# rs-anderson/explicit-alignment-for-vqa-tasks

Hardware: AMD Instinct MI355X
Metric: mapper_train_samples_per_sec (higher is better)
Workload: dtype bf16; 1 GPU; cfg2: CLIP ViT-B/32 -> GPT-2-large (774M), MLP mapper, prefix 10, CC-shaped synthetic batches; per-GPU batch 64, S=42; fwd+bwd+AdamW; random-init weights; global_batch=64, seq_len=42, parallelism=dp1

## Files before the change

### explicit-alignment-for-vqa-tasks_amd/_lib.py

```python
from __future__ import annotations

import ctypes as C
import os

_HERE = os.path.dirname(os.path.abspath(__file__))
LIB_PATH = os.path.join(_HERE, "csrc", "libeavqa_hip.so")

F32, BF16 = 0, 1
ACT = {"none": 0, "tanh": 1, "relu": 2, "gelu_new": 3, "quick_gelu": 4}

i32, i64, f32, ptr = C.c_int, C.c_int64, C.c_float, C.c_void_p

SIGNATURES = {
    "eavqa_abi_version": [],
    "eavqa_strerror": [i32],
    "eavqa_check_device": [],
    "eavqa_gemm": [i32, i32, i32, i32, i32, i32, ptr, i64, ptr, i64, ptr, i64, i32, f32, ptr, i32, ptr, ptr, i64, ptr, i64, ptr],
    "eavqa_layernorm_fwd": [i32, i32, i32, i32, ptr, i64, ptr, ptr, f32, ptr, i64, ptr, ptr, ptr],
    "eavqa_layernorm_bwd": [i32, i32, i32, i32, ptr, i64, ptr, i64, ptr, ptr, ptr, ptr, ptr, i64, ptr, ptr, ptr, i64, ptr],
    "eavqa_layernorm_fwd_fp8": [i32, i32, i32, ptr, i64, ptr, ptr, f32, ptr, i64, ptr, ptr, ptr, ptr],
    "eavqa_layernorm_bwd_fp8": [i32, i32, i32, ptr, i64, ptr, i64, ptr, ptr, ptr, ptr, ptr, i64, ptr, i64, ptr, ptr],
    "eavqa_attention_fwd": [i32, i32, i32, i32, i32, i32, ptr, i64, ptr, i64, ptr, i64, ptr, i64, i64, i64, ptr, i64, ptr, i32, f32, ptr, ptr],
    "eavqa_attention_decode": [i32, i32, i32, i32, i32, ptr, i64, ptr, i64, ptr, i64, i64, ptr, ptr, i64, ptr, i64, ptr, i64, f32, ptr],
    "eavqa_attention_decode_splitk": [i32, i32, i32, i32, i32, ptr, i32, ptr, ptr, i64, ptr, i64, i64, ptr, i64, ptr, i64, f32, ptr],
    "eavqa_attention_bwd": [i32, i32, i32, i32, i32, i32, ptr, i64, ptr, i64, ptr, i64, ptr, i64, ptr, i64,
                            ptr, i64, ptr, i64, ptr, i64, ptr, ptr, i32, f32, ptr, ptr, ptr],
    "eavqa_build_prefix_rows": [i32, i32, i32, ptr, ptr, i32, i32, i32, ptr, ptr, ptr, ptr],
    "eavqa_build_fewshot_rows": [i32, i32, i32, i32, i64, ptr, ptr, i32, ptr, ptr, ptr, ptr, ptr],
    "eavqa_build_row_plan": [i32, i32, i32, ptr, ptr, ptr, ptr, ptr, ptr, ptr, ptr, ptr, ptr],
    "eavqa_copy_rows": [i32, i32, i32, i32, ptr, i64, i64, ptr, i64, i64, i64, ptr],
    "eavqa_transpose": [i32, i32, i32, ptr, i64, ptr, i64, ptr],
    "eavqa_select_rows": [i32, ptr, i32, ptr, ptr, ptr, ptr],
    "eavqa_move_rows": [i32, i32, i32, i32, ptr, i64, ptr, ptr, i64, ptr],
    "eavqa_l2_normalize_rows": [i32, i32, ptr, i64, ptr],
    "eavqa_topk_rows": [i32, i32, ptr, i64, i32, ptr, ptr, ptr],
    "eavqa_gemm_splitk_plan": [i32, i32, i32],
    "eavqa_gemm_splitk": [i32, i32, i32, i32, ptr, i64, ptr, i64, ptr, i32, ptr],
    "eavqa_splitk_finish": [i32, i32, i32, ptr, i32, ptr, i32, ptr, i64, i32, i32, ptr, i64, ptr, i64, ptr, i64, ptr],
    "eavqa_layernorm_splitk": [i32, i32, i32, ptr, i64, ptr, i32, ptr, ptr, i64, ptr, ptr, f32, ptr, i64, ptr],
    "eavqa_gemm_fp8_splitk_plan": [i32, i32, i32],
    "eavqa_gemm_fp8_splitk": [i32, i32, i32, ptr, i64, ptr, ptr, i64, f32, ptr, i32, ptr],
    "eavqa_layernorm_splitk_fp8": [i32, i32, ptr, i64, ptr, i32, ptr, ptr, i64, ptr, ptr, f32, ptr, i64, ptr, ptr],
    "eavqa_rmsnorm_splitk": [i32, i32, i32, ptr, i64, ptr, i32, ptr, i64, ptr, f32, ptr, i64, ptr],
    "eavqa_splitk_finish_gated": [i32, i32, i32, ptr, i32, i32, ptr, i64, ptr],
    "eavqa_attention_decode_splitk_rel": [i32, i32, i32, i32, i32, ptr, i32, i32, ptr, i64, ptr, i64, i64, ptr, i64, ptr, i64, f32, ptr, i64, i32, ptr],
    "eavqa_colsum": [i32, i32, i32, ptr, i64, ptr, i32, ptr],
    "eavqa_embed_assemble": [i32, i32, i32, ptr, ptr, ptr, i64, ptr, i64, ptr, i64, ptr, i64, ptr],
    "eavqa_embed_assemble_bwd": [i32, i32, i32, ptr, ptr, i64, ptr, i64, ptr],
    "eavqa_build_labels": [i32, i32, i32, i32, ptr, i64, i64, ptr, ptr],
    "eavqa_ce_fwd": [i32, i32, i32, ptr, i64, ptr, ptr, ptr, ptr, ptr, ptr],
    "eavqa_guard_count": [ptr, i32, ptr, ptr],
    "eavqa_ce_bwd": [i32, i32, i32, i32, ptr, i64, ptr, ptr, ptr, ptr, ptr, i64, ptr],
    "eavqa_greedy_pick": [i32, i32, ptr, i64, i64, i64, ptr, ptr, i64, ptr, ptr, ptr, ptr],
    "eavqa_adamw": [i64, ptr, ptr, ptr, ptr, i32, f32, f32, f32, f32, f32, f32, i32, ptr, ptr],
    "eavqa_patchify": [i32, i32, i32, i32, ptr, ptr, i64, ptr],
    "eavqa_vit_assemble": [i32, i32, i32, i32, ptr, i64, ptr, ptr, ptr, i64, ptr],
    "eavqa_cast_rows": [i32, i32, i64, ptr, i64, ptr, i64, ptr],
    "eavqa_quantize_rows_fp8": [i32, i32, i32, ptr, i64, ptr, i64, ptr, ptr],
    "eavqa_rmsnorm_fwd": [i32, i32, i32, i32, ptr, i64, ptr, f32, ptr, i64, ptr, ptr],
    "eavqa_rmsnorm_bwd": [i32, i32, i32, i32, ptr, i64, ptr, i64, ptr, ptr, ptr, ptr, i64, ptr, i64, ptr],
    "eavqa_gated_act_fwd": [i32, i32, i32, i32, ptr, i64, ptr, i64, ptr],
    "eavqa_gated_act_bwd": [i32, i32, i32, i32, ptr, i64, ptr, i64, ptr, i64, ptr],
    "eavqa_attention_fwd_rel": [i32, i32, i32, i32, i32, i32, ptr, i64, ptr, i64, ptr, i64, ptr, i64, i64, i64, ptr, i64, i32, f32, ptr, i64, i32, ptr, ptr],
    "eavqa_attention_bwd_rel": [i32, i32, i32, i32, i32, i32, ptr, i64, ptr, i64, ptr, i64, ptr, i64, ptr, i64, ptr, i64, ptr, i64, ptr, i64,
                                ptr, i32, f32, ptr, i64, i32, ptr, ptr, ptr],
    "eavqa_gemm_fp8": [i32, i32, i32, ptr, i64, ptr, ptr, i64, f32, ptr, i64, i32, f32, ptr, i32, ptr, ptr, i64, ptr, i64, ptr, i32],
}
class LMLayer(C.Structure):
    _fields_ = [(n, C.c_void_p) for n in ("ln1_g", "ln1_b", "w_qkv", "b_qkv", "w_o", "b_o", "ln2_g", "ln2_b", "w_fc1", "b_fc1",
                                          "w_fc2", "b_fc2", "k_cache", "v_cache")]


class LMLayerScales(C.Structure):
    _fields_ = [(n, C.c_float) for n in ("s_qkv", "s_o", "s_fc1", "s_fc2")]


class T5DecLayer(C.Structure):
    _fields_ = [(n, C.c_void_p) for n in ("ln_sa", "w_qkv", "w_o", "ln_ca", "w_q_ca", "w_o_ca", "ln_ff", "w_i", "w_o_ff", "k_cache", "v_cache",
                                          "cross_kv")]


class DecodeGemm(C.Structure):
    _fields_ = [("M", i32), ("N", i32), ("K", i32), ("A", ptr), ("lda", i64), ("a_kind", i32), ("gamma", ptr), ("beta", ptr), ("eps", f32),
                ("stats_in", ptr), ("n_stats_in", i32), ("stats_in_cols", i32), ("B", ptr), ("ldb", i64), ("gated_rows", i32),
                ("bias", ptr), ("act", i32), ("residual", ptr), ("ld_residual", i64), ("out_f32", i32), ("n_seg", i32),
                ("out", ptr * 3), ("ld_out", i64 * 3), ("stats_out", ptr)]


class GemmLn(C.Structure):
    _fields_ = [("copy_out", ptr), ("ld_copy", i64), ("stats_out", ptr), ("stats_ld", i32), ("ln_stats", ptr), ("ln_parts", i32),
                ("ln_ld", i32), ("ln_cols", i32), ("ln_c", ptr), ("ln_eps", f32), ("mean_out", ptr), ("rstd_out", ptr)]


SIGNATURES["eavqa_gemm_ln"] = SIGNATURES["eavqa_gemm"][:-1] + [C.POINTER(GemmLn), ptr]
SIGNATURES["eavqa_gemm_decode_cols"] = [i32, i32, i32, i32, i32]
SIGNATURES["eavqa_gemm_decode"] = [C.POINTER(DecodeGemm), ptr]
SIGNATURES["eavqa_t5_decoder_step_workspace_bytes"] = [i32, i32, i32, i32, i32, i32]
SIGNATURES["eavqa_t5_decoder_step"] = [i32, i32, C.POINTER(T5DecLayer), ptr, i32, i32, i32, i32, i32, i32, f32, i32, i32, i32, i32, ptr, ptr, ptr, i64,
                                       ptr, i64, i32, ptr, i64, ptr]
SIGNATURES["eavqa_lm_block_workspace_bytes"] = [i32, i32, i32, i32]
SIGNATURES["eavqa_lm_block_fp8_workspace_bytes"] = [i32, i32, i32]
SIGNATURES["eavqa_lm_block_forward_fp8"] = [i32, C.POINTER(LMLayer), C.POINTER(LMLayerScales), i32, i32, i32, i32, f32, i32, i32, i32, i32, ptr, ptr, i64, ptr, i64, ptr]
SIGNATURES["eavqa_lm_block_forward"] = [i32, i32, C.POINTER(LMLayer), i32, i32, i32, i32, f32, i32, i32, i32, i32, ptr, ptr, i64, ptr, i64, ptr]

SIGNATURES["eavqa_gemm_ex"] = SIGNATURES["eavqa_gemm"] + [i32]
SIGNATURES["eavqa_gemm_ln_ex"] = SIGNATURES["eavqa_gemm_ln"] + [i32]
SIGNATURES["eavqa_attention_fwd_ex"] = SIGNATURES["eavqa_attention_fwd"] + [i32]
SIGNATURES["eavqa_attention_bwd_ex"] = SIGNATURES["eavqa_attention_bwd"] + [i32]
SIGNATURES["eavqa_gemm_splitk_ex"] = SIGNATURES["eavqa_gemm_splitk"] + [i32]
SIGNATURES["eavqa_lm_block_forward_ex"] = SIGNATURES["eavqa_lm_block_forward"] + [i32]
SIGNATURES["eavqa_gemm_decode_ex"] = SIGNATURES["eavqa_gemm_decode"] + [i32]
SIGNATURES["eavqa_t5_decoder_step_ex"] = SIGNATURES["eavqa_t5_decoder_step"] + [i32]

_RESTYPES = {"eavqa_strerror": C.c_char_p, "eavqa_lm_block_workspace_bytes": C.c_int64, "eavqa_lm_block_fp8_workspace_bytes": C.c_int64, "eavqa_t5_decoder_step_workspace_bytes": C.c_int64}

_lib = None


class EavqaError(RuntimeError):
    pass


def load() -> C.CDLL:
    global _lib
    if _lib is not None:
        return _lib
    if not os.path.exists(LIB_PATH):
        raise EavqaError(
            f"{LIB_PATH} is missing: the HIP extension is the only compute path. "
            "Build it with `python -m eavqa_amd.build` (needs hipcc, no GPU required to compile)."
        )
    import torch
    lib = C.CDLL(LIB_PATH)
    for name, argtypes in SIGNATURES.items():
        fn = getattr(lib, name)
        fn.argtypes = argtypes
        fn.restype = _RESTYPES.get(name, C.c_int)
    got = lib.eavqa_abi_version()
    if got != 1:
        raise EavqaError(f"libeavqa_hip.so ABI version {got}, host code expects 1")
    _lib = lib
    return lib


def call(name: str, *args) -> None:
    lib = load()
    rc = getattr(lib, name)(*args)
    if rc != 0:
        raise EavqaError(f"{name} failed: {lib.eavqa_strerror(rc).decode()} (code {rc})")
```

### explicit-alignment-for-vqa-tasks_amd/build.py

```python
from __future__ import annotations

import hashlib
import json
import os
import shutil
import subprocess
import sys
from concurrent.futures import ThreadPoolExecutor

PKG_DIR = os.path.dirname(os.path.abspath(__file__))
CSRC = os.path.join(PKG_DIR, "csrc")
ROOT = os.path.dirname(PKG_DIR)
INCLUDE = os.path.join(ROOT, "include")
OBJ = os.path.join(CSRC, "_obj")
LIB = os.path.join(CSRC, "libeavqa_hip.so")
EXPORTS = os.path.join(CSRC, "exports.map")

HIP_SOURCES = ["gemm.hip", "norm.hip", "attention.hip", "seq.hip", "loss.hip", "optim.hip", "decode.hip", "decode_direct.hip", "retrieval.hip"]
CPP_SOURCES = ["api.cpp", "lm_block.cpp", "t5_block.cpp"]
ARCH = "gfx950"


def _hipcc() -> str:
    exe = shutil.which("hipcc") or "/opt/rocm/bin/hipcc"
    if not os.path.exists(exe):
        raise RuntimeError("hipcc not found: libeavqa_hip.so cannot be built")
    return exe


def _newer(dst: str, deps) -> bool:
    if not os.path.exists(dst):
        return False
    t = os.path.getmtime(dst)
    return all(os.path.getmtime(d) <= t for d in deps)


FLAGS = ["-O3", "-std=c++17", "-fPIC", "-Xarch_host", "-fvisibility=hidden"]


def _digest(rel_paths, extra: str) -> str:
    h = hashlib.sha256(extra.encode())
    for p in rel_paths:
        h.update(p.encode())
        with open(os.path.join(ROOT, p), "rb") as f:
            h.update(f.read())
    return h.hexdigest()


def _read_deps(dfile: str):
    with open(dfile) as f:
        text = f.read().replace("\\\n", " ")
    deps = [os.path.abspath(t) for t in text.split(":", 1)[1].split()]
    return sorted({os.path.relpath(d, ROOT) for d in deps if d.startswith(ROOT + os.sep)})


def _compile(src: str, verbose: bool) -> str:
    stem = os.path.splitext(src)[0]
    obj, dfile, kfile = (os.path.join(OBJ, stem + ext) for ext in (".o", ".d", ".key.json"))
    path = os.path.join(CSRC, src)
    flags = FLAGS + [f"--offload-arch={ARCH}"] + ([] if src.endswith(".hip") else ["-x", "hip"])
    cmd = [_hipcc()] + flags + [f"-I{INCLUDE}", f"-I{CSRC}", "-MD", "-MF", dfile, "-c", path, "-o", obj]
    if os.path.exists(obj) and os.path.exists(kfile):
        try:
            with open(kfile) as f:
                key = json.load(f)
            if key["digest"] == _digest(key["deps"], " ".join(flags)):
                return obj
        except (OSError, KeyError, ValueError):
            pass
    if verbose:
        print(" ".join(cmd), flush=True)
    r = subprocess.run(cmd, capture_output=True, text=True)
    if r.returncode != 0:
        raise RuntimeError(f"hipcc failed on {src}:\n{r.stdout}\n{r.stderr}")
    deps = _read_deps(dfile)
    with open(kfile, "w") as f:
        json.dump({"deps": deps, "digest": _digest(deps, " ".join(flags))}, f)
    return obj


def build(verbose: bool = False, force: bool = False) -> str:
    os.makedirs(OBJ, exist_ok=True)
    if force:
        for f in os.listdir(OBJ):
            os.remove(os.path.join(OBJ, f))
    srcs = HIP_SOURCES + CPP_SOURCES
    with ThreadPoolExecutor(max_workers=min(4, len(srcs))) as ex:
        objs = list(ex.map(lambda s: _compile(s, verbose), srcs))
    if not _newer(LIB, objs + [EXPORTS]):
        cmd = [_hipcc(), f"--offload-arch={ARCH}", "-shared", "-fPIC", f"-Wl,--version-script={EXPORTS}", "-o", LIB] + objs
        if verbose:
            print(" ".join(cmd), flush=True)
        r = subprocess.run(cmd, capture_output=True, text=True)
        if r.returncode != 0:
            raise RuntimeError(f"link failed:\n{r.stdout}\n{r.stderr}")
    return LIB


if __name__ == "__main__":
    print(build(verbose=True, force="--force" in sys.argv))
```

### explicit-alignment-for-vqa-tasks_amd/csrc/gemm.hip

```cpp
#include "common.h"

namespace {

struct Knobs {
    int stagger;
    int ablate;
    bool disable_fast;
    int k64_mode;
    int big_mode;
    int deep;
    int shape_mode;
    int group_n;
    bool no_row_split;
    explicit Knobs(int k = 0) : stagger(k & 15), ablate((k >> 4) & 7), disable_fast(((k >> 7) & 1) != 0), k64_mode((k >> 8) & 63),
                                big_mode((k >> 14) & 3), deep((k >> 16) & 3), shape_mode((k >> 18) & 7), group_n((k >> 21) & 15),
                                no_row_split(((k >> 25) & 1) != 0) {}
};

struct GemmParamsBase {
    const void* A; const void* B; void* C;
    const float* bias; const void* aux_in; void* aux_out; const void* residual;
    const float* row_scale;
    int M, N, K;
    int64_t lda, ldb, ldc, ld_aux, ldr;
    int act, out_f32, res_lowp;
    int out_f16;
    int ablate;
    float alpha;
    int tiles_m, tiles_n;
    int group_n;
    int vec_c, vec_aux, vec_res, vec_bias;
};
struct GemmParams : GemmParamsBase {
    void* copy_out = nullptr; int64_t ld_copy = 0; int vec_copy = 0;
    float* stats_out = nullptr; int stats_ld = 0;
    const float* ln_stats = nullptr; int ln_parts = 0, ln_ld = 0;
    const float* ln_c = nullptr; float ln_inv_n = 0.f, ln_eps = 0.f;
    float* mean_out = nullptr; float* rstd_out = nullptr;
};
constexpr int LN_ROWSTAT_BYTES = 2048;
inline int ln_lds(const GemmParams& p) { return p.ln_stats ? LN_ROWSTAT_BYTES : 0; }
__device__ __forceinline__ GemmParams widen(const GemmParams& k) { return k; }
__device__ __forceinline__ GemmParams widen(const GemmParamsBase& k) { GemmParams p; static_cast<GemmParamsBase&>(p) = k; return p; }
template <bool LNX> struct KernArg { using type = GemmParamsBase; };
template <> struct KernArg<true> { using type = GemmParams; };

constexpr int BM = 128, BN = 128;
constexpr int CS_PITCH = 132;
constexpr int CS_BYTES = BM * CS_PITCH * 4;

__device__ __forceinline__ void tile_coords(const GemmParams& p, int& tm, int& tn) {
    const int nwg = p.tiles_m * p.tiles_n;
    const int bid = blockIdx.x;
    const int q = nwg >> 3, r = nwg & 7, xcd = bid & 7;
    const int wgid = (xcd < r ? xcd * (q + 1) : r * (q + 1) + (xcd - r) * q) + (bid >> 3);
    tm = wgid % p.tiles_m;
    tn = wgid / p.tiles_m;
}

__device__ __forceinline__ void ln_rowstat_fill(const GemmParams& p, float2* rowstat, int m0, int n0, int rows, int tid, int nthreads) {
    if (!p.ln_stats) return;
    for (int r = tid; r < rows; r += nthreads) {
        const int m = min(m0 + r, p.M - 1);
        const float2* q = reinterpret_cast<const float2*>(p.ln_stats) + (int64_t)m * p.ln_ld;
        float s = 0.f, ss = 0.f;
        if (((p.ln_ld | p.ln_parts) & 1) == 0 && (reinterpret_cast<uintptr_t>(p.ln_stats) & 15) == 0) {
            const float4* q4 = reinterpret_cast<const float4*>(q);
            const int n4 = p.ln_parts >> 1;
            for (int i = 0; i < n4; i += 4) {
                float4 t[4];
#pragma unroll
                for (int k = 0; k < 4; ++k) t[k] = q4[min(i + k, n4 - 1)];
#pragma unroll
                for (int k = 0; k < 4; ++k) {
                    const float w = (i + k < n4) ? 1.f : 0.f;
                    s += w * (t[k].x + t[k].z);
                    ss += w * (t[k].y + t[k].w);
                }
            }
        } else {
            for (int i = 0; i < p.ln_parts; ++i) { const float2 t = q[i]; s += t.x; ss += t.y; }
        }
        const float mean = s * p.ln_inv_n;
        const float rstd = 1.0f / sqrtf(fmaxf(ss * p.ln_inv_n - mean * mean, 0.f) + p.ln_eps);
        rowstat[r] = make_float2(rstd, -rstd * mean);
        if (n0 == 0 && m0 + r < p.M && p.mean_out) { p.mean_out[m] = mean; p.rstd_out[m] = rstd; }
    }
}

template <int TPR_, int RPP_, int NPASS_, int PITCH_, int ROWS_ = RPP_ * NPASS_, int LN_UNROLL_ = 4> struct EpiGeo {
    static constexpr int TPR = TPR_, RPP = RPP_, NPASS = NPASS_, PITCH = PITCH_, ROWS = ROWS_;
    static constexpr int LN_UNROLL = LN_UNROLL_;
};
using EpiGeo128 = EpiGeo<32, 8, 16, CS_PITCH>;

template <typename T, int ACT, int MODE, bool FULL, bool LNX>
__device__ __forceinline__ void epilogue_quad(const GemmParams& p, int m, int n, float (&v)[4], const float (&bias4)[4], const float2 rs,
                                              const float (&c4)[4]) {
    const T* aux_in = reinterpret_cast<const T*>(p.aux_in);
    T* aux_out = reinterpret_cast<T*>(p.aux_out);
    const bool full = FULL || (n + 3 < p.N);
    const float al = p.row_scale ? p.alpha * p.row_scale[m] : p.alpha;
    if (LNX && p.ln_stats) {
#pragma unroll
        for (int j = 0; j < 4; ++j) v[j] = (al * rs.x) * v[j] + (bias4[j] + rs.y * c4[j]);
    } else {
#pragma unroll
        for (int j = 0; j < 4; ++j) v[j] = al * v[j] + bias4[j];
    }
    if (aux_out) {
        T* q = aux_out + (int64_t)m * p.ld_aux + n;
        if (FULL || (full && p.vec_aux)) elem<T>::st4(q, make_float4(v[0], v[1], v[2], v[3]));
        else
            for (int j = 0; j < 4; ++j)
                if (n + j < p.N) elem<T>::st(q + j, v[j]);
    }
    if (MODE == 2) {
        const T* q = aux_in + (int64_t)m * p.ld_aux + n;
        float u[4] = {0.f, 0.f, 0.f, 0.f};
        if (FULL || (full && p.vec_aux)) { float4 t = elem<T>::ld4(q); u[0] = t.x; u[1] = t.y; u[2] = t.z; u[3] = t.w; }
        else
            for (int j = 0; j < 4; ++j)
                if (n + j < p.N) u[j] = elem<T>::ld(q + j);
#pragma unroll
        for (int j = 0; j < 4; ++j) v[j] *= act_bwd(ACT, u[j]);
    } else if (MODE == 1) {
#pragma unroll
        for (int j = 0; j < 4; ++j) v[j] = act_fwd(ACT, v[j]);
    }
    if (p.residual) {
        if (p.res_lowp == 2) {
            const f16_t* q = reinterpret_cast<const f16_t*>(p.residual) + (int64_t)m * p.ldr + n;
            if (FULL || (full && p.vec_res)) { float4 t = elem<f16_t>::ld4(q); v[0] += t.x; v[1] += t.y; v[2] += t.z; v[3] += t.w; }
            else
                for (int j = 0; j < 4; ++j)
                    if (n + j < p.N) v[j] += elem<f16_t>::ld(q + j);
        } else if (p.res_lowp) {
            const T* q = reinterpret_cast<const T*>(p.residual) + (int64_t)m * p.ldr + n;
            if (FULL || (full && p.vec_res)) { float4 t = elem<T>::ld4(q); v[0] += t.x; v[1] += t.y; v[2] += t.z; v[3] += t.w; }
            else
                for (int j = 0; j < 4; ++j)
                    if (n + j < p.N) v[j] += elem<T>::ld(q + j);
        } else {
            const float* q = reinterpret_cast<const float*>(p.residual) + (int64_t)m * p.ldr + n;
            if (FULL || (full && p.vec_res)) { float4 t = *reinterpret_cast<const float4*>(q); v[0] += t.x; v[1] += t.y; v[2] += t.z; v[3] += t.w; }
            else
                for (int j = 0; j < 4; ++j)
                    if (n + j < p.N) v[j] += q[j];
        }
    }
    if (p.out_f32) {
        float* q = reinterpret_cast<float*>(p.C) + (int64_t)m * p.ldc + n;
        if (FULL || (full && p.vec_c)) *reinterpret_cast<float4*>(q) = make_float4(v[0], v[1], v[2], v[3]);
        else
            for (int j = 0; j < 4; ++j)
                if (n + j < p.N) q[j] = v[j];
    } else if (p.out_f16) {
        f16_t* q = reinterpret_cast<f16_t*>(p.C) + (int64_t)m * p.ldc + n;
        if (FULL || (full && p.vec_c)) elem<f16_t>::st4(q, make_float4(v[0], v[1], v[2], v[3]));
        else
            for (int j = 0; j < 4; ++j)
                if (n + j < p.N) elem<f16_t>::st(q + j, v[j]);
    } else {
        T* q = reinterpret_cast<T*>(p.C) + (int64_t)m * p.ldc + n;
        if (FULL || (full && p.vec_c)) elem<T>::st4(q, make_float4(v[0], v[1], v[2], v[3]));
        else
            for (int j = 0; j < 4; ++j)
                if (n + j < p.N) elem<T>::st(q + j, v[j]);
    }
    if (LNX && p.copy_out) {
        T* q = reinterpret_cast<T*>(p.copy_out) + (int64_t)m * p.ld_copy + n;
        if (full && p.vec_copy) elem<T>::st4(q, make_float4(v[0], v[1], v[2], v[3]));
        else
            for (int j = 0; j < 4; ++j)
                if (n + j < p.N) elem<T>::st(q + j, v[j]);
    }
}

template <bool FULL>
__device__ __forceinline__ void load_bias4(const GemmParams& p, int n, float (&bias4)[4]) {
    bias4[0] = bias4[1] = bias4[2] = bias4[3] = 0.f;
    if (p.bias) {
        if (FULL) { const float4 b = *reinterpret_cast<const float4*>(p.bias + n); bias4[0] = b.x; bias4[1] = b.y; bias4[2] = b.z; bias4[3] = b.w; }
        else {
#pragma unroll
            for (int j = 0; j < 4; ++j)
                if (n + j < p.N) bias4[j] = p.bias[n + j];
        }
    }
}

struct LnArgs { const float2* rowstat; int row_base; };

template <typename T, int ACT, int MODE, bool FULL, typename G, bool LNX>
__device__ __forceinline__ void epilogue_body(const GemmParams& p, float* Cs, int m0, int n0, const LnArgs ln) {
    const int tid = threadIdx.x;
    if (G::ROWS != G::RPP * G::NPASS && tid >= G::TPR * G::RPP) return;
    const int c4 = (tid % G::TPR) * 4;
    const int n = n0 + c4;
    float bias4[4], lc4[4] = {0.f, 0.f, 0.f, 0.f};
    load_bias4<FULL>(p, n, bias4);
    if (LNX && p.ln_stats) {
#pragma unroll
        for (int j = 0; j < 4; ++j)
            if (FULL || n + j < p.N) lc4[j] = p.ln_c[n + j];
    }
    auto one_pass = [&](int pass) {
        const int row = (tid / G::TPR) + pass * G::RPP;
        const int m = m0 + row;
        if (G::ROWS != G::RPP * G::NPASS && row >= G::ROWS) return;
        if (!FULL && (m >= p.M || n >= p.N)) return;
        const float4 a = *reinterpret_cast<const float4*>(&Cs[row * G::PITCH + c4]);
        float v[4] = {a.x, a.y, a.z, a.w};
        const float2 rs = (LNX && p.ln_stats) ? ln.rowstat[ln.row_base + row] : make_float2(1.f, 0.f);
        epilogue_quad<T, ACT, MODE, FULL, LNX>(p, m, n, v, bias4, rs, lc4);
        if (LNX && p.stats_out) {
            if (!FULL) {
#pragma unroll
                for (int j = 0; j < 4; ++j)
                    if (n + j >= p.N) v[j] = 0.f;
            }
            *reinterpret_cast<float4*>(&Cs[row * G::PITCH + c4]) = make_float4(v[0], v[1], v[2], v[3]);
        }
    };
    if constexpr (LNX && G::LN_UNROLL == 1) {
#pragma unroll 1
        for (int pass = 0; pass < G::NPASS; ++pass) one_pass(pass);
    } else {
#pragma unroll 4
        for (int pass = 0; pass < G::NPASS; ++pass) one_pass(pass);
    }
}

template <typename G>
__device__ __forceinline__ void epilogue_row_sums(const GemmParams& p, const float* Cs, int m0, int n0) {
    constexpr int COLS = G::TPR * 4;
    static_assert(COLS >= 64 && COLS % 4 == 0, "a tile covers at least one 64-column slot");
    __syncthreads();
    const int cols = min(COLS, p.N - n0);
    const int slot0 = n0 / 64, slot1 = (n0 + COLS < p.N) ? (n0 + COLS) / 64 : p.stats_ld;
    for (int r = threadIdx.x; r < G::ROWS; r += blockDim.x) {
        const int m = m0 + r;
        if (m >= p.M) continue;
        float s = 0.f, ss = 0.f;
        for (int c = 0; c < cols; c += 4) {
            const float4 t = *reinterpret_cast<const float4*>(&Cs[r * G::PITCH + c]);
            s += (t.x + t.y) + (t.z + t.w);
            ss += (t.x * t.x + t.y * t.y) + (t.z * t.z + t.w * t.w);
        }
        float2* q = reinterpret_cast<float2*>(p.stats_out) + (int64_t)m * p.stats_ld;
        q[slot0] = make_float2(s, ss);
        for (int i = slot0 + 1; i < slot1; ++i) q[i] = make_float2(0.f, 0.f);
    }
}

template <typename T, int ACT, int MODE, typename G, bool LNX>
__device__ __forceinline__ void epilogue_mode(const GemmParams& p, float* Cs, int m0, int n0, const LnArgs ln) {
    constexpr int ROWS = G::ROWS, COLS = G::TPR * 4;
    const bool full_tile = (m0 + ROWS <= p.M) && (n0 + COLS <= p.N) && p.vec_c && (!(p.aux_in || p.aux_out) || p.vec_aux) &&
                           (!p.residual || p.vec_res) && (!p.bias || p.vec_bias);
    if (full_tile) epilogue_body<T, ACT, MODE, true, G, LNX>(p, Cs, m0, n0, ln);
    else epilogue_body<T, ACT, MODE, false, G, LNX>(p, Cs, m0, n0, ln);
    if (LNX && p.stats_out) epilogue_row_sums<G>(p, Cs, m0, n0);
}

template <typename T, typename G = EpiGeo128, bool LNX = true>
__device__ __forceinline__ void epilogue(const GemmParams& p, float* Cs, int m0, int n0, const LnArgs ln = LnArgs{nullptr, 0}) {
    const int mode = p.aux_in ? 2 : (p.act != EAVQA_ACT_NONE ? 1 : 0);
    if (mode == 0) { epilogue_mode<T, EAVQA_ACT_NONE, 0, G, LNX>(p, Cs, m0, n0, ln); return; }
    switch (p.act) {
        case EAVQA_ACT_TANH:
            if (mode == 1) epilogue_mode<T, EAVQA_ACT_TANH, 1, G, LNX>(p, Cs, m0, n0, ln); else epilogue_mode<T, EAVQA_ACT_TANH, 2, G, LNX>(p, Cs, m0, n0, ln);
            break;
        case EAVQA_ACT_RELU:
            if (mode == 1) epilogue_mode<T, EAVQA_ACT_RELU, 1, G, LNX>(p, Cs, m0, n0, ln); else epilogue_mode<T, EAVQA_ACT_RELU, 2, G, LNX>(p, Cs, m0, n0, ln);
            break;
        case EAVQA_ACT_GELU_NEW:
            if (mode == 1) epilogue_mode<T, EAVQA_ACT_GELU_NEW, 1, G, LNX>(p, Cs, m0, n0, ln); else epilogue_mode<T, EAVQA_ACT_GELU_NEW, 2, G, LNX>(p, Cs, m0, n0, ln);
            break;
        case EAVQA_ACT_QUICK_GELU:
            if (mode == 1) epilogue_mode<T, EAVQA_ACT_QUICK_GELU, 1, G, LNX>(p, Cs, m0, n0, ln); else epilogue_mode<T, EAVQA_ACT_QUICK_GELU, 2, G, LNX>(p, Cs, m0, n0, ln);
            break;
        default:
            epilogue_mode<T, EAVQA_ACT_NONE, 0, G, LNX>(p, Cs, m0, n0, ln);
    }
}

template <typename T, typename G = EpiGeo128>
__device__ __forceinline__ void epilogue_any(const GemmParams& p, float* Cs, int m0, int n0, const LnArgs ln = LnArgs{nullptr, 0}) {
    if (p.ln_stats || p.stats_out || p.copy_out) epilogue<T, G, true>(p, Cs, m0, n0, ln);
    else epilogue<T, G, false>(p, Cs, m0, n0, ln);
}


constexpr int BK16 = 64;
constexpr int OPER16_BYTES = 128 * BK16 * 2;

__device__ __forceinline__ int swz16(int row, int kc) { return row * 128 + ((kc ^ (row & 7)) << 4); }

template <bool KC>
__device__ __forceinline__ void g2r_16(uint4 (&r)[4], const bf16_t* X, int64_t ld, int row0, int rows_max,
                                       int k0, int K) {
    const int tid = threadIdx.x;
#pragma unroll
    for (int i = 0; i < 4; ++i) {
        const int c = tid + 256 * i;
        uint4 v = make_uint4(0u, 0u, 0u, 0u);
        if (KC) {
            const int row = c >> 3, kc = c & 7;
            const int gr = row0 + row, gk = k0 + kc * 8;
            if (gr < rows_max && gk < K) v = *reinterpret_cast<const uint4*>(X + (int64_t)gr * ld + gk);
        } else {
            const int k = c >> 4, rc = c & 15;
            const int gk = k0 + k, gr = row0 + rc * 8;
            if (gk < K && gr < rows_max) v = *reinterpret_cast<const uint4*>(X + (int64_t)gk * ld + gr);
        }
        r[i] = v;
    }
}
template <bool KC>
__device__ __forceinline__ void r2s_16(const uint4 (&r)[4], char* S) {
    const int tid = threadIdx.x;
#pragma unroll
    for (int i = 0; i < 4; ++i) {
        const int c = tid + 256 * i;
        if (KC) {
// ... 612 lines not shown
inline int big_grid(int tiles_m, int tiles_n, int& gx, int& gy) {
    int best_gx = 8, best_cost = 1 << 30, best_rounds = 1 << 30;
    const int cand[4] = {8, 4, 2, 1};
    for (int c = 0; c < 4; ++c) {
        const int x = cand[c], y = 8 / x;
        const int pm = (tiles_m + x - 1) / x, pn = (tiles_n + y - 1) / y;
        const int rounds = (pm * pn + 31) / 32, cost = pm + pn;
        if (rounds < best_rounds || (rounds == best_rounds && cost < best_cost)) { best_rounds = rounds; best_cost = cost; best_gx = x; }
    }
    gx = best_gx; gy = 8 / gx;
    return ((tiles_m + gx - 1) / gx) * ((tiles_n + gy - 1) / gy);
}

int launch_big(const GemmParams& p, hipStream_t stream) {
    static std::atomic<bool> configured{false};
    if (!configured.load(std::memory_order_acquire)) {
        if (hipFuncSetAttribute(reinterpret_cast<const void*>(gemm_bf16_big_kernel<false>), hipFuncAttributeMaxDynamicSharedMemorySize,
                                GLDS_BYTES) != hipSuccess ||
            hipFuncSetAttribute(reinterpret_cast<const void*>(gemm_bf16_big_kernel<true>), hipFuncAttributeMaxDynamicSharedMemorySize,
                                GLDS_BYTES + LN_ROWSTAT_BYTES) != hipSuccess)
            return EAVQA_E_LAUNCH;
        configured.store(true, std::memory_order_release);
    }
    const int tiles_m = (p.M + GBM - 1) / GBM, tiles_n = (p.N + GBN - 1) / GBN;
    int gx, gy;
    const int per_xcd = big_grid(tiles_m, tiles_n, gx, gy);
    if (p.ln_stats || p.stats_out || p.copy_out)
        hipLaunchKernelGGL(gemm_bf16_big_kernel<true>, dim3(per_xcd * 8), dim3(1024), GLDS_BYTES + ln_lds(p), stream, p, gx, gy, tiles_m, tiles_n);
    else
        hipLaunchKernelGGL(gemm_bf16_big_kernel<false>, dim3(per_xcd * 8), dim3(1024), GLDS_BYTES, stream, p, gx, gy, tiles_m, tiles_n);
    EAVQA_LAUNCH_CHECK();
    return EAVQA_OK;
}

inline int big_split_rows(int M, int N) {
    const int rem = M % GBM;
    if (rem == 0 || rem > 192 || M <= GBM) return 0;
    int gx, gy;
    const int tiles_n = (N + GBN - 1) / GBN;
    const int with = (big_grid((M + GBM - 1) / GBM, tiles_n, gx, gy) + 31) / 32, without = (big_grid(M / GBM, tiles_n, gx, gy) + 31) / 32;
    return without < with ? rem : 0;
}

bool use_big(const GemmParams& p, const Knobs& kn) {
    if (p.K % GBK) return false;
    if (kn.big_mode == 1) return false;
    if (kn.big_mode == 2) return true;
    const int tiles = ((p.M + GBM - 1) / GBM) * ((p.N + GBN - 1) / GBN);
    return tiles >= 144;
}


#include "gemm_k64.hip"

inline float k64_cost(const GemmParams& p, const K64Choice& c, float* multi_round_loop = nullptr) {
    const int tiles_m = (p.M + c.bm - 1) / c.bm, tiles_n = (p.N + c.bn - 1) / c.bn;
    const GridPlan g = plan_grid(tiles_m, tiles_n, c.bm, c.bn);
    const float rounds = float((g.per_xcd + 31) / 32);
    const float loop = rounds * c.rate * (c.bm + c.bn) * (p.K / 64);
    if (multi_round_loop) *multi_round_loop = rounds > 1.f ? loop : 0.f;
    return loop + rounds * 0.1f * c.bm * c.bn + 4500.f;
}

#include "gemm_fp8.hip"

template <int MF>
__global__ __launch_bounds__(512) void gemm_bf16_skinny_kernel(GemmParams p) {
    __shared__ float red[8][64][17];
    const int tid = threadIdx.x, lane = tid & 63, wave = tid >> 6;
    const int x = lane & 15, g = lane >> 4;
    const int n0 = blockIdx.x * 16;
    const bf16_t* A = reinterpret_cast<const bf16_t*>(p.A);
    const bf16_t* B = reinterpret_cast<const bf16_t*>(p.B);
    const int nsteps = p.K >> 5;
    const int per_wave = (nsteps + 7) >> 3;
    const int s_begin = wave * per_wave, s_end = min(nsteps, s_begin + per_wave);
    const bf16_t* bp = B + (int64_t)min(n0 + x, p.N - 1) * p.ldb + 8 * g;
    const bf16_t* ap[MF];
#pragma unroll
    for (int f = 0; f < MF; ++f) ap[f] = A + (int64_t)min(16 * f + x, p.M - 1) * p.lda + 8 * g;
    f32x4 acc[MF];
#pragma unroll
    for (int f = 0; f < MF; ++f) acc[f] = (f32x4){0.f, 0.f, 0.f, 0.f};

    int s = s_begin;
    for (; s + 8 <= s_end; s += 8) {
        bf16x8 b[8], a[8][MF];
#pragma unroll
        for (int u = 0; u < 8; ++u) {
            b[u] = *reinterpret_cast<const bf16x8*>(bp + (s + u) * 32);
#pragma unroll
            for (int f = 0; f < MF; ++f) a[u][f] = *reinterpret_cast<const bf16x8*>(ap[f] + (s + u) * 32);
        }
#pragma unroll
        for (int u = 0; u < 8; ++u)
#pragma unroll
            for (int f = 0; f < MF; ++f) acc[f] = __builtin_amdgcn_mfma_f32_16x16x32_bf16(a[u][f], b[u], acc[f], 0, 0, 0);
    }
    for (; s < s_end; ++s) {
        const bf16x8 b = *reinterpret_cast<const bf16x8*>(bp + s * 32);
#pragma unroll
        for (int f = 0; f < MF; ++f) {
            const bf16x8 a = *reinterpret_cast<const bf16x8*>(ap[f] + s * 32);
            acc[f] = __builtin_amdgcn_mfma_f32_16x16x32_bf16(a, b, acc[f], 0, 0, 0);
        }
    }
#pragma unroll
    for (int f = 0; f < MF; ++f)
#pragma unroll
        for (int r = 0; r < 4; ++r) red[wave][16 * f + 4 * g + r][x] = acc[f][r];
    __syncthreads();
    for (int e = tid; e < MF * 16 * 16; e += 512) {
        const int m = e >> 4, c = e & 15, n = n0 + c;
        if (m >= p.M || n >= p.N) continue;
        float v = 0.f;
#pragma unroll
        for (int w = 0; w < 8; ++w) v += red[w][m][c];
        v = p.alpha * v + (p.bias ? p.bias[n] : 0.f);
        const int64_t ia = (int64_t)m * p.ld_aux + n;
        if (p.aux_out) elem<bf16_t>::st(reinterpret_cast<bf16_t*>(p.aux_out) + ia, v);
        if (p.aux_in) v *= act_bwd(p.act, elem<bf16_t>::ld(reinterpret_cast<const bf16_t*>(p.aux_in) + ia));
        else v = act_fwd(p.act, v);
        if (p.residual) v += p.res_lowp == 2 ? elem<f16_t>::ld(reinterpret_cast<const f16_t*>(p.residual) + (int64_t)m * p.ldr + n)
                             : p.res_lowp ? elem<bf16_t>::ld(reinterpret_cast<const bf16_t*>(p.residual) + (int64_t)m * p.ldr + n)
                                          : reinterpret_cast<const float*>(p.residual)[(int64_t)m * p.ldr + n];
        if (p.out_f32) reinterpret_cast<float*>(p.C)[(int64_t)m * p.ldc + n] = v;
        else if (p.out_f16) elem<f16_t>::st(reinterpret_cast<f16_t*>(p.C) + (int64_t)m * p.ldc + n, v);
        else elem<bf16_t>::st(reinterpret_cast<bf16_t*>(p.C) + (int64_t)m * p.ldc + n, v);
    }
}

int launch_skinny(const GemmParams& p, hipStream_t stream) {
    const int blocks = (p.N + 15) / 16;
    const int mf = (p.M + 15) / 16;
    if (mf == 1) hipLaunchKernelGGL(gemm_bf16_skinny_kernel<1>, dim3(blocks), dim3(512), 0, stream, p);
    else if (mf == 2) hipLaunchKernelGGL(gemm_bf16_skinny_kernel<2>, dim3(blocks), dim3(512), 0, stream, p);
    else if (mf == 3) hipLaunchKernelGGL(gemm_bf16_skinny_kernel<3>, dim3(blocks), dim3(512), 0, stream, p);
    else hipLaunchKernelGGL(gemm_bf16_skinny_kernel<4>, dim3(blocks), dim3(512), 0, stream, p);
    EAVQA_LAUNCH_CHECK();
    return EAVQA_OK;
}

constexpr int BK32 = 16;
constexpr int PITCH32 = 17;
constexpr int OPER32_FLOATS = 128 * PITCH32;

template <bool KC>
__device__ __forceinline__ void g2r_32(float4 (&r)[2], const float* X, int64_t ld, int row0, int rows_max,
                                       int k0, int K) {
    const int tid = threadIdx.x;
#pragma unroll
    for (int i = 0; i < 2; ++i) {
        const int c = tid + 256 * i;
        float4 v = make_float4(0.f, 0.f, 0.f, 0.f);
        if (KC) {
            const int row = c >> 2, kc = c & 3;
            const int gr = row0 + row, gk = k0 + kc * 4;
            if (gr < rows_max && gk < K) v = *reinterpret_cast<const float4*>(X + (int64_t)gr * ld + gk);
        } else {
            const int k = c >> 5, rc = c & 31;
            const int gk = k0 + k, gr = row0 + rc * 4;
            if (gk < K && gr < rows_max) v = *reinterpret_cast<const float4*>(X + (int64_t)gk * ld + gr);
        }
        r[i] = v;
    }
}
template <bool KC>
__device__ __forceinline__ void r2s_32(const float4 (&r)[2], float* S) {
    const int tid = threadIdx.x;
#pragma unroll
    for (int i = 0; i < 2; ++i) {
        const int c = tid + 256 * i;
        const float w[4] = {r[i].x, r[i].y, r[i].z, r[i].w};
        if (KC) {
            const int row = c >> 2, kc = c & 3;
#pragma unroll
            for (int j = 0; j < 4; ++j) S[row * PITCH32 + kc * 4 + j] = w[j];
        } else {
            const int k = c >> 5, rc = c & 31;
#pragma unroll
            for (int j = 0; j < 4; ++j) S[(rc * 4 + j) * PITCH32 + k] = w[j];
        }
    }
}

template <bool A_KC, bool B_KC>
__global__ __launch_bounds__(256) void gemm_f32_kernel(GemmParams p) {
    extern __shared__ __attribute__((aligned(16))) char smem[];
    float* sm = reinterpret_cast<float*>(smem);
    float* const As0 = sm;
    float* const Bs0 = sm + 2 * OPER32_FLOATS;

    int tm, tn;
    tile_coords(p, tm, tn);
    const int m0 = tm * BM, n0 = tn * BN;
    const int tid = threadIdx.x, lane = tid & 63, wave = tid >> 6;
    const int wm = wave >> 1, wn = wave & 1;
    const float* A = reinterpret_cast<const float*>(p.A);
    const float* B = reinterpret_cast<const float*>(p.B);

    f32x16 acc[2][2];
#pragma unroll
    for (int i = 0; i < 2; ++i)
#pragma unroll
        for (int j = 0; j < 2; ++j)
#pragma unroll
            for (int r = 0; r < 16; ++r) acc[i][j][r] = 0.f;

    const int nk = (p.K + BK32 - 1) / BK32;
    float4 ra[2], rb[2];
    g2r_32<A_KC>(ra, A, p.lda, m0, p.M, 0, p.K);
    g2r_32<B_KC>(rb, B, p.ldb, n0, p.N, 0, p.K);
    r2s_32<A_KC>(ra, As0);
    r2s_32<B_KC>(rb, Bs0);
    __syncthreads();

    const int frow = lane & 31, fk = lane >> 5;
    for (int kt = 0; kt < nk; ++kt) {
        const int cur = kt & 1;
        if (kt + 1 < nk) {
            g2r_32<A_KC>(ra, A, p.lda, m0, p.M, (kt + 1) * BK32, p.K);
            g2r_32<B_KC>(rb, B, p.ldb, n0, p.N, (kt + 1) * BK32, p.K);
        }
        const float* Ac = As0 + cur * OPER32_FLOATS;
        const float* Bc = Bs0 + cur * OPER32_FLOATS;
#pragma unroll
        for (int s = 0; s < BK32 / 2; ++s) {
            float af[2], bfr[2];
#pragma unroll
            for (int i = 0; i < 2; ++i) af[i] = Ac[(wm * 64 + i * 32 + frow) * PITCH32 + s * 2 + fk];
#pragma unroll
            for (int j = 0; j < 2; ++j) bfr[j] = Bc[(wn * 64 + j * 32 + frow) * PITCH32 + s * 2 + fk];
#pragma unroll
            for (int i = 0; i < 2; ++i)
#pragma unroll
                for (int j = 0; j < 2; ++j)
                    acc[i][j] = __builtin_amdgcn_mfma_f32_32x32x2f32(af[i], bfr[j], acc[i][j], 0, 0, 0);
        }
        if (kt + 1 < nk) {
            r2s_32<A_KC>(ra, As0 + (cur ^ 1) * OPER32_FLOATS);
            r2s_32<B_KC>(rb, Bs0 + (cur ^ 1) * OPER32_FLOATS);
        }
        __syncthreads();
    }

    float* Cs = reinterpret_cast<float*>(smem);
#pragma unroll
    for (int i = 0; i < 2; ++i)
#pragma unroll
        for (int j = 0; j < 2; ++j)
#pragma unroll
            for (int r = 0; r < 16; ++r) {
                const int row = wm * 64 + i * 32 + (r & 3) + 8 * (r >> 2) + 4 * (lane >> 5);
                const int col = wn * 64 + j * 32 + (lane & 31);
                Cs[row * CS_PITCH + col] = acc[i][j][r];
            }
    float2* rowstat = reinterpret_cast<float2*>(smem + CS_BYTES);
    ln_rowstat_fill(p, rowstat, m0, n0, BM, tid, 256);
    __syncthreads();
    if constexpr (A_KC && B_KC) epilogue_any<float>(p, Cs, m0, n0, LnArgs{rowstat, 0});
    else epilogue<float, EpiGeo128, false>(p, Cs, m0, n0);
}

typedef void (*gemm_kernel_t)(GemmParams);

int launch(gemm_kernel_t kernel, const GemmParams& p, hipStream_t stream) {
    static std::atomic<gemm_kernel_t> configured[8];
    bool done = false;
    for (int i = 0; i < 8; ++i) done |= (configured[i].load(std::memory_order_acquire) == kernel);
    if (!done) {
        if (hipFuncSetAttribute(reinterpret_cast<const void*>(kernel), hipFuncAttributeMaxDynamicSharedMemorySize,
                                CS_BYTES + LN_ROWSTAT_BYTES) != hipSuccess)
            return EAVQA_E_LAUNCH;
        for (int i = 0; i < 8; ++i) {
            gemm_kernel_t expected = nullptr;
            if (configured[i].compare_exchange_strong(expected, kernel, std::memory_order_acq_rel) || expected == kernel) break;
        }
    }
    const int nwg = p.tiles_m * p.tiles_n;
    hipLaunchKernelGGL(kernel, dim3(nwg), dim3(256), CS_BYTES + ln_lds(p), stream, p);
    EAVQA_LAUNCH_CHECK();
    return EAVQA_OK;
}


}

namespace {
eavqa_gemm_ln_t ln_rows_from(const eavqa_gemm_ln_t& x, int64_t r0, size_t esz) {
    eavqa_gemm_ln_t y = x;
    if (x.copy_out) y.copy_out = static_cast<char*>(x.copy_out) + (size_t)r0 * (size_t)x.ld_copy * esz;
    if (x.stats_out) y.stats_out = x.stats_out + (size_t)r0 * (size_t)x.stats_ld * 2;
    if (x.ln_stats) y.ln_stats = x.ln_stats + (size_t)r0 * (size_t)x.ln_ld * 2;
    if (x.mean_out) y.mean_out = x.mean_out + r0;
    if (x.rstd_out) y.rstd_out = x.rstd_out + r0;
    return y;
}

int gemm_impl(int dtype, int a_kc, int b_kc, int M, int N, int K,
              const void* A, int64_t lda, const void* B, int64_t ldb,
              void* C, int64_t ldc, int out_flags, float alpha,
              const float* bias, int act,
              const void* aux_in, void* aux_out, int64_t ld_aux,
              const void* residual, int64_t ldr, const eavqa_gemm_ln_t* ln, void* stream, int knobs) {
    const Knobs kn(knobs);
    const bool ln_consumer = ln && ln->ln_stats;
    if (ln) {
        if (ln->copy_out && ln->ld_copy < N) return EAVQA_E_ARG;
        if (ln->stats_out && ln->stats_ld < (N + 63) / 64) return EAVQA_E_ARG;
        if (ln_consumer && (!ln->ln_c || ln->ln_parts <= 0 || ln->ln_ld < ln->ln_parts || ln->ln_cols <= 0 || !(ln->ln_eps >= 0.f))) return EAVQA_E_ARG;
        if ((ln->mean_out != nullptr) != (ln->rstd_out != nullptr) || (ln->mean_out && !ln_consumer)) return EAVQA_E_ARG;
        if (!(a_kc && b_kc)) return EAVQA_E_SHAPE;
    }
    if (out_flags & ~(EAVQA_GEMM_OUT_F32 | EAVQA_GEMM_RESIDUAL_LOWP | EAVQA_GEMM_STREAM_F16)) return EAVQA_E_ARG;
    if ((out_flags & (EAVQA_GEMM_RESIDUAL_LOWP | EAVQA_GEMM_STREAM_F16)) && dtype != EAVQA_BF16) return EAVQA_E_DTYPE;
    const int out_f32 = out_flags & EAVQA_GEMM_OUT_F32;
    const int stream_f16 = (out_flags & EAVQA_GEMM_STREAM_F16) != 0;
    const int res_lowp = (out_flags & EAVQA_GEMM_RESIDUAL_LOWP) ? (stream_f16 ? 2 : 1) : 0;
    if (!A || !B || !C) return EAVQA_E_ARG;
    if (M <= 0 || N <= 0 || K <= 0) return EAVQA_E_ARG;
    if (dtype != EAVQA_F32 && dtype != EAVQA_BF16) return EAVQA_E_DTYPE;
    if (act < EAVQA_ACT_NONE || act > EAVQA_ACT_QUICK_GELU) return EAVQA_E_DTYPE;
    const int vec = dtype == EAVQA_BF16 ? 8 : 4;
    const int a_contig = a_kc ? K : M, b_contig = b_kc ? K : N;
    if (a_contig % vec || b_contig % vec) return EAVQA_E_SHAPE;
    if (lda % vec || ldb % vec) return EAVQA_E_ALIGN;
    if (!eavqa_aligned16(A) || !eavqa_aligned16(B)) return EAVQA_E_ALIGN;
    if (lda < a_contig || ldb < b_contig || ldc < N) return EAVQA_E_ARG;
    if ((aux_in || aux_out) && ld_aux < N) return EAVQA_E_ARG;
    if (residual && ldr < N) return EAVQA_E_ARG;

    GemmParams p;
    p.A = A; p.B = B; p.C = C; p.bias = bias; p.aux_in = aux_in; p.aux_out = aux_out; p.residual = residual; p.row_scale = nullptr; p.ablate = kn.ablate;
    p.M = M; p.N = N; p.K = K; p.lda = lda; p.ldb = ldb; p.ldc = ldc; p.ld_aux = ld_aux; p.ldr = ldr;
    p.act = act; p.out_f32 = out_f32; p.res_lowp = res_lowp; p.out_f16 = stream_f16 && !out_f32; p.alpha = alpha;
    p.group_n = kn.group_n == 0 ? BIG_GROUP_N : kn.group_n - 1;
    p.tiles_m = (M + BM - 1) / BM;
    p.tiles_n = (N + BN - 1) / BN;
    const int esz = dtype == EAVQA_BF16 ? 2 : 4;
    auto vec_ok = [](const void* ptr, int64_t ld, int bytes_per_elem) {
        return ((reinterpret_cast<uintptr_t>(ptr) % (4 * bytes_per_elem)) == 0) && (ld % 4 == 0);
    };
    p.vec_c = vec_ok(C, ldc, out_f32 ? 4 : esz);
    p.vec_aux = vec_ok(aux_in ? aux_in : aux_out, ld_aux, esz);
    p.vec_res = vec_ok(residual, ldr, res_lowp ? esz : 4);
    p.vec_bias = (reinterpret_cast<uintptr_t>(bias) % 16) == 0;
    if (ln) {
        p.copy_out = ln->copy_out; p.ld_copy = ln->ld_copy; p.vec_copy = ln->copy_out ? vec_ok(ln->copy_out, ln->ld_copy, esz) : 0;
        p.stats_out = ln->stats_out; p.stats_ld = ln->stats_ld;
        if (ln_consumer) {
            p.ln_stats = ln->ln_stats; p.ln_parts = ln->ln_parts; p.ln_ld = ln->ln_ld; p.ln_c = ln->ln_c;
            p.ln_inv_n = 1.0f / float(ln->ln_cols); p.ln_eps = ln->ln_eps; p.mean_out = ln->mean_out; p.rstd_out = ln->rstd_out;
        }
    }
    hipStream_t s = reinterpret_cast<hipStream_t>(stream);
    if (dtype == EAVQA_BF16) {
        if (a_kc && b_kc && (K % 64) == 0 && kn.k64_mode >= 2 && kn.k64_mode < 2 + N_K64) return K64_SHAPES[kn.k64_mode - 2].launch(p, s);
        const bool few_columns = kn.k64_mode == 0 && kn.shape_mode == 0 && kn.big_mode == 0 && N <= 4096;
        if (!ln && a_kc && b_kc && !kn.disable_fast && M <= 64 && (K % 32) == 0 && N >= 64 && (kn.k64_mode == 1 || (K % 64) != 0 || few_columns)) return launch_skinny(p, s);
        const int big_rem = (a_kc && b_kc && kn.big_mode != 1 && !kn.no_row_split) ? big_split_rows(M, N) : 0;
        const float big_split_ns = big_rem ? 12000.f : 0.f;
        auto run_big = [&](const GemmParams& pp) -> int {
            if (!big_rem) return launch_big(pp, s);
            GemmParams p1 = pp;
            p1.M = M - big_rem;
            p1.tiles_m = (p1.M + BM - 1) / BM;
            const int rc1 = launch_big(p1, s);
            if (rc1) return rc1;
            const int64_t r0 = M - big_rem;
            const size_t ces = out_f32 ? 4 : 2, res_es = res_lowp ? 2 : 4;
            auto off = [](const void* base, int64_t rows, int64_t ld, size_t es) -> const void* {
                return base ? static_cast<const char*>(base) + (size_t)rows * (size_t)ld * es : nullptr;
            };
            eavqa_gemm_ln_t ln2;
            if (ln) ln2 = ln_rows_from(*ln, r0, 2);
            return gemm_impl(dtype, a_kc, b_kc, big_rem, N, K, off(A, r0, lda, 2), lda, B, ldb, const_cast<void*>(off(C, r0, ldc, ces)), ldc, out_flags,
                             alpha, bias, act, off(aux_in, r0, ld_aux, 2), const_cast<void*>(off(aux_out, r0, ld_aux, 2)), ld_aux,
                             off(residual, r0, ldr, res_es), ldr, ln ? &ln2 : nullptr, stream, 0);
        };
        int bgx, bgy;
        const int big_rounds = (big_grid((M - big_rem + GBM - 1) / GBM, (N + GBN - 1) / GBN, bgx, bgy) + 31) / 32;
        const bool many_big_tiles = big_rounds >= 4 || (big_rounds >= 2 && (M + GBM - 1) / GBM > 96);
        if (a_kc && b_kc && !kn.disable_fast && (K % 64) == 0 && kn.k64_mode != 1 && kn.shape_mode == 0 && kn.big_mode == 0 && !many_big_tiles) {
            int pick = K64_AUTO[0];
            float best_loop = 0.f;
            float best = k64_cost(p, K64_SHAPES[pick], &best_loop);
            for (int i = 1; i < N_K64_AUTO; ++i) {
                float loop;
                const float c = k64_cost(p, K64_SHAPES[K64_AUTO[i]], &loop);
                if (c < best) { best = c; pick = K64_AUTO[i]; best_loop = loop; }
            }
            best += 0.35f * best_loop;
            const float big_cost = float(big_rounds) * (float(K / 64) * (big_rounds == 1 ? 1380.f : 1530.f) + 9000.f) + 3000.f + big_split_ns;
            if (M > 64 && big_cost < best) return run_big(p);
            return K64_SHAPES[pick].launch(p, s);
        }
        if (a_kc && b_kc && !kn.disable_fast && (K % FBK) == 0 && !ln) {
            if (kn.shape_mode >= 2 && kn.shape_mode < 7) return SHAPES[kn.shape_mode - 2].launch(p, s);
            const bool big_ok = (K % GBK) == 0 && kn.big_mode != 1;
            if (big_ok && kn.big_mode == 2) return run_big(p);
            float best = tile_cost(p, 128, 128, RATE_FAST);
            int pick = -1;
            if (big_ok && use_big(p, kn)) {
                GemmParams pf = p;
                pf.M = M - big_rem;
                best = fminf(best, tile_cost(pf, 256, 256, RATE_BIG) + big_split_ns);
                pick = -2;
            }
            if (kn.shape_mode != 1)
                for (int i = 0; i < 5; ++i) {
                    const float c = tile_cost(p, SHAPES[i].bm, SHAPES[i].bn, SHAPES[i].rate);
                    if (c < best * 0.95f) { best = c; pick = i; }
                }
            if (pick >= 0) return SHAPES[pick].launch(p, s);
            if (pick == -2) return run_big(p);
            return launch_fast(p, s, kn);
        }
        if (a_kc && b_kc) return launch(gemm_bf16_kernel<true, true>, p, s);
        if (a_kc && !b_kc) return launch(gemm_bf16_kernel<true, false>, p, s);
        if (!a_kc && b_kc) return launch(gemm_bf16_kernel<false, true>, p, s);
        return launch(gemm_bf16_kernel<false, false>, p, s);
    }
    if (a_kc && b_kc) return launch(gemm_f32_kernel<true, true>, p, s);
    if (a_kc && !b_kc) return launch(gemm_f32_kernel<true, false>, p, s);
    if (!a_kc && b_kc) return launch(gemm_f32_kernel<false, true>, p, s);
    return launch(gemm_f32_kernel<false, false>, p, s);
}
}

extern "C" int eavqa_gemm_ex(int dtype, int a_kc, int b_kc, int M, int N, int K,
                             const void* A, int64_t lda, const void* B, int64_t ldb,
                             void* C, int64_t ldc, int out_flags, float alpha,
                             const float* bias, int act,
                             const void* aux_in, void* aux_out, int64_t ld_aux,
                             const void* residual, int64_t ldr, void* stream, int knobs) {
    return gemm_impl(dtype, a_kc, b_kc, M, N, K, A, lda, B, ldb, C, ldc, out_flags, alpha, bias, act, aux_in, aux_out, ld_aux, residual, ldr,
                     nullptr, stream, knobs);
}

extern "C" int eavqa_gemm_ln_ex(int dtype, int a_kc, int b_kc, int M, int N, int K,
                                const void* A, int64_t lda, const void* B, int64_t ldb,
                                void* C, int64_t ldc, int out_flags, float alpha,
                                const float* bias, int act,
                                const void* aux_in, void* aux_out, int64_t ld_aux,
                                const void* residual, int64_t ldr, const eavqa_gemm_ln_t* ln, void* stream, int knobs) {
    if (!ln) return EAVQA_E_ARG;
    return gemm_impl(dtype, a_kc, b_kc, M, N, K, A, lda, B, ldb, C, ldc, out_flags, alpha, bias, act, aux_in, aux_out, ld_aux, residual, ldr,
                     ln, stream, knobs);
}

extern "C" int eavqa_gemm_ln(int dtype, int a_kc, int b_kc, int M, int N, int K,
                             const void* A, int64_t lda, const void* B, int64_t ldb,
                             void* C, int64_t ldc, int out_flags, float alpha,
                             const float* bias, int act,
                             const void* aux_in, void* aux_out, int64_t ld_aux,
                             const void* residual, int64_t ldr, const eavqa_gemm_ln_t* ln, void* stream) {
    return eavqa_gemm_ln_ex(dtype, a_kc, b_kc, M, N, K, A, lda, B, ldb, C, ldc, out_flags, alpha, bias, act, aux_in, aux_out, ld_aux, residual,
                            ldr, ln, stream, 0);
}

extern "C" int eavqa_gemm(int dtype, int a_kc, int b_kc, int M, int N, int K,
                          const void* A, int64_t lda, const void* B, int64_t ldb,
                          void* C, int64_t ldc, int out_flags, float alpha,
                          const float* bias, int act,
                          const void* aux_in, void* aux_out, int64_t ld_aux,
                          const void* residual, int64_t ldr, void* stream) {
    return eavqa_gemm_ex(dtype, a_kc, b_kc, M, N, K, A, lda, B, ldb, C, ldc, out_flags, alpha, bias, act, aux_in, aux_out, ld_aux,
                         residual, ldr, stream, 0);
}

extern "C" int eavqa_quantize_rows_fp8(int dtype, int rows, int cols, const void* x, int64_t ldx, void* out, int64_t ld_out,
                                       float* row_scale, void* stream) {
    if (!x || !out || !row_scale || rows <= 0 || cols <= 0) return EAVQA_E_ARG;
    if (cols % 4) return EAVQA_E_SHAPE;
    if (ldx % 4 || ld_out % 4 || ldx < cols || ld_out < cols) return EAVQA_E_ALIGN;
    if ((reinterpret_cast<uintptr_t>(x) & 7u) || (reinterpret_cast<uintptr_t>(out) & 3u)) return EAVQA_E_ALIGN;
    hipStream_t s = reinterpret_cast<hipStream_t>(stream);
    const bool reg_ok = dtype == EAVQA_BF16 && cols % 8 == 0 && cols <= 16384 && ldx % 8 == 0 && ld_out % 8 == 0 &&
                        !(reinterpret_cast<uintptr_t>(x) & 15u) && !(reinterpret_cast<uintptr_t>(out) & 7u);
    if (reg_ok) {
        const int nv = (cols / 8 + 255) / 256;
#define EAVQA_QR(NV) hipLaunchKernelGGL(quantize_rows_fp8_reg_kernel<NV>, dim3(rows), dim3(256), 0, s, cols, reinterpret_cast<const bf16_t*>(x), \
                                        ldx, reinterpret_cast<unsigned char*>(out), ld_out, row_scale)
        if (nv <= 1) EAVQA_QR(1); else if (nv <= 2) EAVQA_QR(2); else if (nv <= 4) EAVQA_QR(4); else EAVQA_QR(8);
#undef EAVQA_QR
    } else if (dtype == EAVQA_BF16)
        hipLaunchKernelGGL(quantize_rows_fp8_kernel<bf16_t>, dim3(rows), dim3(256), 0, s, cols, reinterpret_cast<const bf16_t*>(x), ldx,
                           reinterpret_cast<unsigned char*>(out), ld_out, row_scale);
    else if (dtype == EAVQA_F32)
        hipLaunchKernelGGL(quantize_rows_fp8_kernel<float>, dim3(rows), dim3(256), 0, s, cols, reinterpret_cast<const float*>(x), ldx,
                           reinterpret_cast<unsigned char*>(out), ld_out, row_scale);
    else return EAVQA_E_DTYPE;
    EAVQA_LAUNCH_CHECK();
    return EAVQA_OK;
}

extern "C" int eavqa_gemm_fp8(int M, int N, int K, const void* A, int64_t lda, const float* a_row_scale, const void* B, int64_t ldb,
                              float b_scale, void* C, int64_t ldc, int out_f32, float alpha, const float* bias, int act,
                              const void* aux_in, void* aux_out, int64_t ld_aux, const float* residual, int64_t ldr, void* stream, int tile) {
    if (!A || !B || !C || !a_row_scale) return EAVQA_E_ARG;
    if (M <= 0 || N <= 0 || K <= 0) return EAVQA_E_ARG;
    if (act < EAVQA_ACT_NONE || act > EAVQA_ACT_QUICK_GELU) return EAVQA_E_DTYPE;
    if (K % 128) return EAVQA_E_SHAPE;
    if (lda % 16 || ldb % 16 || !eavqa_aligned16(A) || !eavqa_aligned16(B)) return EAVQA_E_ALIGN;
    if (lda < K || ldb < K || ldc < N) return EAVQA_E_ARG;
    if ((aux_in || aux_out) && ld_aux < N) return EAVQA_E_ARG;
    if (residual && ldr < N) return EAVQA_E_ARG;
    GemmParams p;
    p.A = A; p.B = B; p.C = C; p.bias = bias; p.aux_in = aux_in; p.aux_out = aux_out; p.residual = residual; p.row_scale = a_row_scale; p.ablate = 0;
    p.M = M; p.N = N; p.K = K; p.lda = lda; p.ldb = ldb; p.ldc = ldc; p.ld_aux = ld_aux; p.ldr = ldr;
    p.act = act; p.out_f32 = out_f32; p.res_lowp = 0; p.out_f16 = 0; p.alpha = alpha * b_scale;
    p.group_n = 0;
    p.tiles_m = (M + BM - 1) / BM;
    p.tiles_n = (N + BN - 1) / BN;
    auto vec_ok = [](const void* ptr, int64_t ld, int bytes_per_elem) {
        return ((reinterpret_cast<uintptr_t>(ptr) % (4 * bytes_per_elem)) == 0) && (ld % 4 == 0);
    };
    p.vec_c = vec_ok(C, ldc, out_f32 ? 4 : 2);
    p.vec_aux = vec_ok(aux_in ? aux_in : aux_out, ld_aux, 2);
    p.vec_res = vec_ok(residual, ldr, 4);
    p.vec_bias = (reinterpret_cast<uintptr_t>(bias) % 16) == 0;
    hipStream_t s = reinterpret_cast<hipStream_t>(stream);
    if (tile > 0 && tile <= N_FP8) return FP8_SHAPES[tile - 1].launch(p, s);
    GemmParams q = p;
    q.K = K / 2;
    int pick = 0;
    float best = k64_cost(q, FP8_SHAPES[0]);
    for (int i = 1; i < N_FP8; ++i) {
        const float c = k64_cost(q, FP8_SHAPES[i]);
        if (c < best) { best = c; pick = i; }
    }
    return FP8_SHAPES[pick].launch(p, s);
}
```

### explicit-alignment-for-vqa-tasks_amd/csrc/gemm_k64.hip

```cpp
template <int N> __device__ __forceinline__ void wait_vm() { __builtin_amdgcn_s_waitcnt(vm_only(N)); }


template <int WM, int WN, int MF, int NF, int NST_, int LW_> struct K64SGeo {
    static constexpr int NST = NST_, LW = LW_;
    static constexpr int NC = WM * WN;
    static constexpr int NT = 64 * (NC + LW);
    static constexpr int TBM = 16 * MF * WM, TBN = 16 * NF * WN;
    static constexpr int PT = (TBM + TBN) / 8;
    static constexpr int P_LO = PT / LW, P_HI = (PT + LW - 1) / LW, N_HI = PT % LW;
    static constexpr int AOPER = TBM * 128, STAGE = (TBM + TBN) * 128, RING = NST * STAGE;
    static constexpr int PITCH = TBN + 4;
    static constexpr int SP = (16 * MF * WM * PITCH * 4 <= RING) ? WM : ((16 * MF * (WM / 2) * PITCH * 4 <= RING && WM >= 2) ? WM / 2 : 1);
    static constexpr int MFC = (16 * MF * PITCH * 4 <= RING) ? MF : MF / 2;
    static constexpr int PROWS = 16 * MFC * SP;
    static constexpr int TPR = TBN / 4;
    static constexpr int RPP = NT / TPR, NPASS = (PROWS + RPP - 1) / RPP;
    static_assert((TBM + TBN) % 8 == 0 && P_LO >= 1, "stage must cut into whole pieces, at least one per loader");
    static_assert(16 * MFC * PITCH * 4 <= RING && MF % MFC == 0 && (MFC == MF || SP == 1), "C staging pass must fit the ring");
    static_assert(WM % SP == 0 && RING <= 160 * 1024 && NT <= 1024, "geometry");
    static_assert(P_HI * (NST - 1) <= 63 && NST >= 2 && NST <= 6, "vmcnt field");
};

template <class G>
__device__ __forceinline__ void k64s_loader_role(const char* A, const char* B, int64_t lda_bytes, int64_t ldb_bytes, int M, int N, int m0,
                                                 int n0, int nk, char* smem, int lw, int lane) {
    constexpr int NST = G::NST;
    const bool hi = lw < G::N_HI;
    const char* src[G::P_HI];
    int dst[G::P_HI];
#pragma unroll
    for (int i = 0; i < G::P_HI; ++i) {
        const int piece = min(lw + G::LW * i, G::PT - 1);
        const int row = piece * 8 + (lane >> 3), slot = lane & 7;
        const int kc = (slot ^ (lane >> 3)) * 16;
        src[i] = row < G::TBM ? A + (int64_t)min(m0 + row, M - 1) * lda_bytes + kc
                              : B + (int64_t)min(n0 + row - G::TBM, N - 1) * ldb_bytes + kc;
        dst[i] = piece * 1024;
    }
    auto issue = [&](int kt, int stage) {
        char* st = smem + stage * G::STAGE;
#pragma unroll
        for (int i = 0; i < G::P_HI; ++i)
            if (i < G::P_LO || hi)
                __builtin_amdgcn_global_load_lds((const __attribute__((address_space(1))) void*)(src[i] + (int64_t)kt * 128),
                                                 (__attribute__((address_space(3))) void*)(st + dst[i]), 16, 0, 0);
    };
    auto wait_tiles = [&](int tiles) {
        if (hi) {
            if (NST >= 6 && tiles >= 5) wait_vm<(NST >= 6 ? 5 : 0) * G::P_HI>();
            else if (NST >= 5 && tiles >= 4) wait_vm<(NST >= 5 ? 4 : 0) * G::P_HI>();
            else if (NST >= 4 && tiles >= 3) wait_vm<(NST >= 4 ? 3 : 0) * G::P_HI>();
            else if (NST >= 3 && tiles >= 2) wait_vm<(NST >= 3 ? 2 : 0) * G::P_HI>();
            else if (tiles >= 1) wait_vm<G::P_HI>();
            else wait_vm<0>();
        } else {
            if (NST >= 6 && tiles >= 5) wait_vm<(NST >= 6 ? 5 : 0) * G::P_LO>();
            else if (NST >= 5 && tiles >= 4) wait_vm<(NST >= 5 ? 4 : 0) * G::P_LO>();
            else if (NST >= 4 && tiles >= 3) wait_vm<(NST >= 4 ? 3 : 0) * G::P_LO>();
            else if (NST >= 3 && tiles >= 2) wait_vm<(NST >= 3 ? 2 : 0) * G::P_LO>();
            else if (tiles >= 1) wait_vm<G::P_LO>();
            else wait_vm<0>();
        }
    };
#pragma unroll
    for (int i = 0; i < NST; ++i)
        if (i < nk) issue(i, i);
    wait_tiles(min(nk, NST) - 1);
    __builtin_amdgcn_s_barrier();
    int stage = 0;
    for (int t = 0; t + 1 < nk; ++t) {
        wait_tiles(min(nk - 1, t + NST - 1) - (t + 1));
        __builtin_amdgcn_s_barrier();
        if (t + NST < nk) issue(t + NST, stage);
        stage = (stage + 1 == NST) ? 0 : stage + 1;
    }
}

template <class G, int WM, int WN, int MF, int NF, bool LNX = false>
__device__ __forceinline__ void k64s_store_tile(const GemmParams& p, const f32x4 (&acc)[MF][NF], char* smem, int wave, int lane, int m0, int n0,
                                                const float2* rowstat = nullptr) {
    const int wm = wave / WN, wn = wave % WN;
    float* Cs = reinterpret_cast<float*>(smem);
    constexpr int CH = MF / G::MFC;
    constexpr int NPASSES = (WM / G::SP) * CH;
    for (int pass = 0; pass < NPASSES; ++pass) {
        const int wgrp = pass / CH, chunk = pass % CH;
        if (wave < G::NC && wm / G::SP == wgrp) {
            const int r0 = (wm % G::SP) * 16 * G::MFC;
#pragma unroll
            for (int i = 0; i < MF; ++i) {
                if (i / G::MFC != chunk) continue;
#pragma unroll
                for (int j = 0; j < NF; ++j)
#pragma unroll
                    for (int r = 0; r < 4; ++r) {
                        const int row = r0 + (i % G::MFC) * 16 + (lane >> 4) * 4 + r;
                        const int col = wn * 16 * NF + j * 16 + (lane & 15);
                        Cs[row * G::PITCH + col] = acc[i][j][r];
                    }
            }
        }
        __syncthreads();
        const int row_base = wgrp * G::SP * 16 * MF + chunk * 16 * G::MFC;
        epilogue<bf16_t, EpiGeo<G::TPR, G::RPP, G::NPASS, G::PITCH, G::PROWS>, LNX>(p, Cs, m0 + row_base, n0, LnArgs{rowstat, row_base});
        if (pass + 1 < NPASSES) __syncthreads();
    }
}

template <int WM, int WN, int MF, int NF, int NST, int LW, bool LNX>
__global__ __launch_bounds__(64 * (WM * WN + LW)) void gemm_bf16_k64s_kernel(typename KernArg<LNX>::type pk, int gx, int gy, int tiles_m, int tiles_n) {
    const GemmParams p = widen(pk);
    using G = K64SGeo<WM, WN, MF, NF, NST, LW>;
    extern __shared__ __attribute__((aligned(16))) char smem[];
    int tm, tn;
    if (!shaped_tile(gx, gy, tiles_m, tiles_n, tm, tn)) return;
    const int m0 = tm * G::TBM, n0 = tn * G::TBN;
    const int tid = threadIdx.x, lane = tid & 63;
    const int wave = __builtin_amdgcn_readfirstlane(tid >> 6);
    if (p.ablate & 4) return;
    const int nk = (p.ablate & 2) ? 1 : (p.K >> 6);
    f32x4 acc[MF][NF];
#pragma unroll
    for (int i = 0; i < MF; ++i)
#pragma unroll
        for (int j = 0; j < NF; ++j) acc[i][j] = (f32x4){0.f, 0.f, 0.f, 0.f};
    const int wm = wave / WN, wn = wave % WN;
    float2* rowstat = reinterpret_cast<float2*>(smem + G::RING);

    if (wave >= G::NC) {
        k64s_loader_role<G>(reinterpret_cast<const char*>(p.A), reinterpret_cast<const char*>(p.B), p.lda * 2, p.ldb * 2, p.M, p.N, m0, n0, nk,
                            smem, wave - G::NC, lane);
    } else {
        const int frow = lane & 15, fk = lane >> 4;
        const int sw0 = ((fk ^ (frow & 7)) << 4);
        const int a_off = (wm * 16 * MF + frow) * 128;
        const int b_off = G::AOPER + (wn * 16 * NF + frow) * 128;
        bf16x8 fa[2][MF], fb[2][NF];
        auto read_frags = [&](int set, const char* st, int sw) {
#pragma unroll
            for (int i = 0; i < MF; ++i) fa[set][i] = *reinterpret_cast<const bf16x8*>(st + a_off + i * 2048 + sw);
#pragma unroll
            for (int j = 0; j < NF; ++j) fb[set][j] = *reinterpret_cast<const bf16x8*>(st + b_off + j * 2048 + sw);
        };
        auto mfma_all = [&](int set) {
#pragma unroll
            for (int i = 0; i < MF; ++i)
#pragma unroll
                for (int j = 0; j < NF; ++j)
                    acc[i][j] = __builtin_amdgcn_mfma_f32_16x16x32_bf16(fa[set][i], fb[set][j], acc[i][j], 0, 0, 0);
        };
        if (LNX) ln_rowstat_fill(p, rowstat, m0, n0, G::TBM, tid, 64 * G::NC);
        __builtin_amdgcn_s_barrier();
        read_frags(0, smem, sw0);
        int stage = 0;
        for (int t = 0; t < nk; ++t) {
            const char* st = smem + stage * G::STAGE;
            const int nstage = (stage + 1 == NST) ? 0 : stage + 1;
            __builtin_amdgcn_sched_barrier(0);
            __builtin_amdgcn_s_waitcnt(0xC07F);
            read_frags(1, st, sw0 ^ 64);
            mfma_all(0);
            __builtin_amdgcn_sched_barrier(0);
            __builtin_amdgcn_s_waitcnt(0xC07F);
            if (t + 1 < nk) {
                __builtin_amdgcn_s_barrier();
                read_frags(0, smem + nstage * G::STAGE, sw0);
            }
            mfma_all(1);
            stage = nstage;
        }
    }
    __syncthreads();
    if (p.ablate & 1) {
        if (acc[0][0][0] == 12345.678f) reinterpret_cast<float*>(p.C)[0] = acc[0][0][0];
        return;
    }
    k64s_store_tile<G, WM, WN, MF, NF, LNX>(p, acc, smem, wave, lane, m0, n0, rowstat);
}

template <int WM, int WN, int MF, int NF, int NST, int LW, bool WITH_LN = false>
int launch_k64s(const GemmParams& p, hipStream_t stream) {
    using G = K64SGeo<WM, WN, MF, NF, NST, LW>;
    const bool ln = p.ln_stats || p.stats_out || p.copy_out;
    if (ln && !WITH_LN) return EAVQA_E_SHAPE;
    static std::atomic<bool> configured{false};
    if (!configured.load(std::memory_order_acquire)) {
        if (hipFuncSetAttribute(reinterpret_cast<const void*>(gemm_bf16_k64s_kernel<WM, WN, MF, NF, NST, LW, false>),
                                hipFuncAttributeMaxDynamicSharedMemorySize, G::RING) != hipSuccess)
            return EAVQA_E_LAUNCH;
        if constexpr (WITH_LN) {
            if (hipFuncSetAttribute(reinterpret_cast<const void*>(gemm_bf16_k64s_kernel<WM, WN, MF, NF, NST, LW, true>),
                                    hipFuncAttributeMaxDynamicSharedMemorySize, G::RING + LN_ROWSTAT_BYTES) != hipSuccess)
                return EAVQA_E_LAUNCH;
        }
        configured.store(true, std::memory_order_release);
    }
    static_assert(!WITH_LN || G::RING + LN_ROWSTAT_BYTES <= 160 * 1024, "ring + row statistics of eavqa_gemm_ln");
    const int tiles_m = (p.M + G::TBM - 1) / G::TBM, tiles_n = (p.N + G::TBN - 1) / G::TBN;
    const GridPlan g = plan_grid(tiles_m, tiles_n, G::TBM, G::TBN);
    if constexpr (WITH_LN) {
        if (ln) {
            hipLaunchKernelGGL((gemm_bf16_k64s_kernel<WM, WN, MF, NF, NST, LW, true>), dim3(g.per_xcd * 8), dim3(G::NT), G::RING + ln_lds(p), stream, p,
                               g.gx, g.gy, tiles_m, tiles_n);
            EAVQA_LAUNCH_CHECK();
            return EAVQA_OK;
        }
    }
    hipLaunchKernelGGL((gemm_bf16_k64s_kernel<WM, WN, MF, NF, NST, LW, false>), dim3(g.per_xcd * 8), dim3(G::NT), G::RING, stream, p, g.gx, g.gy,
                       tiles_m, tiles_n);
    EAVQA_LAUNCH_CHECK();
    return EAVQA_OK;
}

struct K64Choice { int bm, bn, wg_per_cu; float rate; int (*launch)(const GemmParams&, hipStream_t); };
const K64Choice K64_SHAPES[] = {
    {128, 80, 2, 1.1f, launch_k64s<4, 1, 2, 5, 3, 2>},
    {128, 80, 2, 1.1f, launch_k64s<4, 1, 2, 5, 3, 4>},
    {128, 128, 2, 1.1f, launch_k64s<2, 2, 4, 4, 2, 4>},
    {256, 128, 1, 1.97f, launch_k64s<4, 2, 4, 4, 3, 4, true>},
    {256, 160, 1, 1.93f, launch_k64s<4, 2, 4, 5, 3, 4, true>},
    {128, 80, 1, 1.56f, launch_k64s<4, 1, 2, 5, 4, 2, true>},
    {128, 96, 1, 1.1f, launch_k64s<4, 1, 2, 6, 3, 2>},
    {256, 192, 1, 1.1f, launch_k64s<4, 2, 4, 6, 2, 4>},
    {256, 256, 1, 1.1f, launch_k64s<2, 4, 8, 4, 2, 4>},
    {128, 128, 1, 1.73f, launch_k64s<2, 2, 4, 4, 3, 2, true>},
    {128, 256, 1, 1.97f, launch_k64s<2, 4, 4, 4, 3, 4, true>},
};
constexpr int N_K64 = sizeof(K64_SHAPES) / sizeof(K64_SHAPES[0]);
constexpr int K64_AUTO[] = {5, 3, 4, 9, 10};
constexpr int N_K64_AUTO = sizeof(K64_AUTO) / sizeof(K64_AUTO[0]);
```

### explicit-alignment-for-vqa-tasks_amd/models/clip_vit.py

```python
from __future__ import annotations

from dataclasses import dataclass
from typing import Dict

import torch

from .. import ops

Tensor = torch.Tensor


@dataclass
class ViTConfig:
    width: int
    n_layer: int
    n_head: int
    mlp: int
    patch: int
    image: int
    proj: int
    eps: float = 1e-5
    act: str = "quick_gelu"

    @property
    def n_patch(self) -> int:
        return (self.image // self.patch) ** 2


KNOWN_VITS = {
    "ViT-B/32": ViTConfig(768, 12, 12, 3072, 32, 224, 512),
    "ViT-B/16": ViTConfig(768, 12, 12, 3072, 16, 224, 512),
    "ViT-L/14": ViTConfig(1024, 24, 16, 4096, 14, 224, 768),
    "ViT-L/14@336px": ViTConfig(1024, 24, 16, 4096, 14, 336, 768),
}


def random_init_vit_state_dict(cfg: ViTConfig, seed: int = 2021, device="cpu") -> Dict[str, Tensor]:
    g = torch.Generator(device=device).manual_seed(seed)
    W = cfg.width

    def n(*shape, std=0.02):
        return torch.randn(*shape, generator=g, device=device) * std

    ones, zeros = (lambda k: torch.ones(k, device=device)), (lambda k: torch.zeros(k, device=device))
    p = "vision_model."
    sd = {
        p + "embeddings.class_embedding": n(W, std=W ** -0.5),
        p + "embeddings.patch_embedding.weight": n(W, 3, cfg.patch, cfg.patch),
        p + "embeddings.position_embedding.weight": n(cfg.n_patch + 1, W),
        p + "pre_layrnorm.weight": ones(W), p + "pre_layrnorm.bias": zeros(W),
        p + "post_layernorm.weight": ones(W), p + "post_layernorm.bias": zeros(W),
        "visual_projection.weight": n(cfg.proj, W, std=W ** -0.5),
    }
    for i in range(cfg.n_layer):
        q = f"{p}encoder.layers.{i}."
        for nm in ("q_proj", "k_proj", "v_proj", "out_proj"):
            sd[q + f"self_attn.{nm}.weight"], sd[q + f"self_attn.{nm}.bias"] = n(W, W, std=W ** -0.5), zeros(W)
        sd[q + "layer_norm1.weight"], sd[q + "layer_norm1.bias"] = ones(W), zeros(W)
        sd[q + "layer_norm2.weight"], sd[q + "layer_norm2.bias"] = ones(W), zeros(W)
        sd[q + "mlp.fc1.weight"], sd[q + "mlp.fc1.bias"] = n(cfg.mlp, W), zeros(cfg.mlp)
        sd[q + "mlp.fc2.weight"], sd[q + "mlp.fc2.bias"] = n(W, cfg.mlp), zeros(W)
    return sd


class ClipVisionEncoder:

    def __init__(self, cfg: ViTConfig, state_dict: Dict[str, Tensor], dtype: torch.dtype = torch.bfloat16, device="cuda",
                 stream_dtype: torch.dtype = None):
        self.cfg, self.dtype, self.device = cfg, dtype, torch.device(device)
        if stream_dtype is None:
            stream_dtype = torch.float16 if dtype == torch.bfloat16 else torch.float32
        self.stream_dtype = stream_dtype
        if dtype == torch.float32 and stream_dtype != torch.float32:
            raise ValueError("fp32 mode streams in float32")
        if stream_dtype not in (torch.float32, torch.bfloat16, torch.float16):
            raise ValueError("stream_dtype must be float32, bfloat16 or float16")
        T = lambda t: t.to(device=self.device, dtype=dtype).contiguous()
        F = lambda t: t.to(device=self.device, dtype=torch.float32).contiguous()
        p = "vision_model."
        W = cfg.width
        K = 3 * cfg.patch * cfg.patch
        self.kpad = (K + 31) // 32 * 32
        wp = torch.zeros((W, self.kpad), dtype=torch.float32)
        wp[:, :K] = state_dict[p + "embeddings.patch_embedding.weight"].reshape(W, K).float().cpu()
        self.w_patch = T(wp)
        self.cls = F(state_dict[p + "embeddings.class_embedding"])
        self.pos = F(state_dict[p + "embeddings.position_embedding.weight"])
        self.pre_g, self.pre_b = F(state_dict[p + "pre_layrnorm.weight"]), F(state_dict[p + "pre_layrnorm.bias"])
        self.post_g, self.post_b = F(state_dict[p + "post_layernorm.weight"]), F(state_dict[p + "post_layernorm.bias"])
        self.w_proj = T(state_dict["visual_projection.weight"])
        self.layers = []
        for i in range(cfg.n_layer):
            q = f"{p}encoder.layers.{i}."
            self.layers.append(dict(
                ln1_g=F(state_dict[q + "layer_norm1.weight"]), ln1_b=F(state_dict[q + "layer_norm1.bias"]),
                w_qkv=T(torch.cat([state_dict[q + f"self_attn.{n}_proj.weight"] for n in "qkv"], 0)),
                b_qkv=F(torch.cat([state_dict[q + f"self_attn.{n}_proj.bias"] for n in "qkv"], 0)),
                w_o=T(state_dict[q + "self_attn.out_proj.weight"]), b_o=F(state_dict[q + "self_attn.out_proj.bias"]),
                ln2_g=F(state_dict[q + "layer_norm2.weight"]), ln2_b=F(state_dict[q + "layer_norm2.bias"]),
                w_fc1=T(state_dict[q + "mlp.fc1.weight"]), b_fc1=F(state_dict[q + "mlp.fc1.bias"]),
                w_fc2=T(state_dict[q + "mlp.fc2.weight"]), b_fc2=F(state_dict[q + "mlp.fc2.bias"]),
            ))

    @torch.no_grad()
    def encode_image(self, pixels: Tensor) -> Tensor:
        c, T = self.cfg, self.dtype
        B = pixels.shape[0]
        if pixels.shape[-1] != c.image or pixels.shape[-2] != c.image:
            raise ValueError(f"Input image size ({pixels.shape[-2]}*{pixels.shape[-1]}) doesn't match model ({c.image}*{c.image}).")
        W, H, N = c.width, c.n_head, c.n_patch + 1
        hd = W // H
        patches = ops.patchify(pixels.to(self.device), c.patch, T, self.kpad)
        pe = ops.gemm(patches, self.w_patch)
        x = ops.vit_assemble(pe, self.cls, self.pos, B, c.n_patch)
        ST = self.stream_dtype
        x = ops.layernorm_fwd(x, self.pre_g, self.pre_b, c.eps, ST)
        x1 = torch.empty_like(x)
        for L in self.layers:
            a = ops.layernorm_fwd(x, L["ln1_g"], L["ln1_b"], c.eps, T)
            qkv = ops.gemm(a, L["w_qkv"], bias=L["b_qkv"])
            ctx = ops.attention_fwd(qkv[:, :W], qkv[:, W:2 * W], qkv[:, 2 * W:], B, H, N, N, hd, causal=False, scale=hd ** -0.5)
            ops.gemm(ctx, L["w_o"], bias=L["b_o"], residual=x, out=x1)
            a2 = ops.layernorm_fwd(x1, L["ln2_g"], L["ln2_b"], c.eps, T)
            f = ops.gemm(a2, L["w_fc1"], bias=L["b_fc1"], act=c.act)
            ops.gemm(f, L["w_fc2"], bias=L["b_fc2"], residual=x1, out=x)
        pooled = ops.layernorm_fwd(x.view(B, N, W)[:, 0], self.post_g, self.post_b, c.eps, T)
        return ops.gemm(pooled, self.w_proj, out_f32=True)


class EncodeAhead:

    def __init__(self, vit: "ClipVisionEncoder"):
        self.vit = vit
        self.side = torch.cuda.Stream(device=vit.device)

    def submit(self, pixels: Tensor):
        main = torch.cuda.current_stream(self.vit.device)
        self.side.wait_stream(main)
        if pixels.is_cuda:
            pixels.record_stream(self.side)
        with torch.cuda.stream(self.side):
            emb = self.vit.encode_image(pixels)
            done = torch.cuda.Event()
            done.record(self.side)
        return emb, done

    def result(self, ticket) -> Tensor:
        emb, done = ticket
        main = torch.cuda.current_stream(self.vit.device)
        main.wait_event(done)
        emb.record_stream(main)
        return emb
```

### explicit-alignment-for-vqa-tasks_amd/models/lm.py

```python
from __future__ import annotations

import json
import math
import os
from dataclasses import dataclass
from typing import Dict, Optional

import torch

from .. import ops

Tensor = torch.Tensor


@dataclass
class LMConfig:
    arch: str
    n_layer: int
    n_head: int
    n_embd: int
    ffn: int
    vocab: int
    n_pos: int
    eps: float = 1e-5
    act: str = "gelu_new"
    eos_token_id: Optional[int] = None
    pad_token_id: Optional[int] = None

    @property
    def head_dim(self) -> int:
        return self.n_embd // self.n_head

    @property
    def pos_mode(self) -> int:
        return 0 if self.arch == "gpt2" else 1

    @staticmethod
    def from_hf_dict(d: dict) -> "LMConfig":
        mt = d.get("model_type", "gpt2")
        if mt == "gpt2":
            E = d.get("n_embd", 768)
            return LMConfig("gpt2", d.get("n_layer", 12), d.get("n_head", 12), E, d.get("n_inner") or 4 * E,
                            d.get("vocab_size", 50257), d.get("n_positions", 1024), d.get("layer_norm_epsilon", 1e-5),
                            d.get("activation_function", "gelu_new"), d.get("eos_token_id", 50256), d.get("pad_token_id"))
        if mt == "opt":
            E = d.get("hidden_size", 768)
            if d.get("word_embed_proj_dim", E) != E or not d.get("do_layer_norm_before", True):
                raise NotImplementedError("OPT-350m style project_in/out / post-LN is not on the hot path")
            return LMConfig("opt", d.get("num_hidden_layers", 12), d.get("num_attention_heads", 12), E, d.get("ffn_dim", 3072),
                            d.get("vocab_size", 50272), d.get("max_position_embeddings", 2048), 1e-5,
                            d.get("activation_function", "relu"), d.get("eos_token_id", 2), d.get("pad_token_id", 1))
        raise NotImplementedError(f"model_type {mt!r} is not a causal LM on the hot path")


KNOWN_CONFIGS = {
    "gpt2": dict(model_type="gpt2", n_embd=768, n_layer=12, n_head=12, vocab_size=50257, n_positions=1024),
    "gpt2-medium": dict(model_type="gpt2", n_embd=1024, n_layer=24, n_head=16, vocab_size=50257, n_positions=1024),
    "gpt2-large": dict(model_type="gpt2", n_embd=1280, n_layer=36, n_head=20, vocab_size=50257, n_positions=1024),
    "gpt2-xl": dict(model_type="gpt2", n_embd=1600, n_layer=48, n_head=25, vocab_size=50257, n_positions=1024),
    "facebook/opt-125m": dict(model_type="opt", hidden_size=768, num_hidden_layers=12, num_attention_heads=12, ffn_dim=3072),
    "facebook/opt-1.3b": dict(model_type="opt", hidden_size=2048, num_hidden_layers=24, num_attention_heads=32, ffn_dim=8192),
    "facebook/opt-2.7b": dict(model_type="opt", hidden_size=2560, num_hidden_layers=32, num_attention_heads=32, ffn_dim=10240),
    "facebook/opt-6.7b": dict(model_type="opt", hidden_size=4096, num_hidden_layers=32, num_attention_heads=32, ffn_dim=16384),
}


def random_init_state_dict(cfg: LMConfig, seed: int = 2021, device="cpu") -> Dict[str, Tensor]:
    g = torch.Generator(device=device).manual_seed(seed)
    E, F, V = cfg.n_embd, cfg.ffn, cfg.vocab

    def n(*shape, std=0.02):
        return torch.randn(*shape, generator=g, device=device) * std

    sd: Dict[str, Tensor] = {}
    ones, zeros = (lambda k: torch.ones(k, device=device)), (lambda k: torch.zeros(k, device=device))
    if cfg.arch == "gpt2":
        sd["transformer.wte.weight"] = n(V, E)
        sd["transformer.wpe.weight"] = n(cfg.n_pos, E)
        ps = 0.02 / math.sqrt(2 * cfg.n_layer)
        for i in range(cfg.n_layer):
            p = f"transformer.h.{i}."
            sd[p + "ln_1.weight"], sd[p + "ln_1.bias"] = ones(E), zeros(E)
            sd[p + "attn.c_attn.weight"], sd[p + "attn.c_attn.bias"] = n(E, 3 * E), zeros(3 * E)
            sd[p + "attn.c_proj.weight"], sd[p + "attn.c_proj.bias"] = n(E, E, std=ps), zeros(E)
            sd[p + "ln_2.weight"], sd[p + "ln_2.bias"] = ones(E), zeros(E)
            sd[p + "mlp.c_fc.weight"], sd[p + "mlp.c_fc.bias"] = n(E, F), zeros(F)
            sd[p + "mlp.c_proj.weight"], sd[p + "mlp.c_proj.bias"] = n(F, E, std=ps), zeros(E)
        sd["transformer.ln_f.weight"], sd["transformer.ln_f.bias"] = ones(E), zeros(E)
    else:
        pre = "model.decoder."
        sd[pre + "embed_tokens.weight"] = n(V, E)
        sd[pre + "embed_positions.weight"] = n(cfg.n_pos + 2, E)
        for i in range(cfg.n_layer):
            p = f"{pre}layers.{i}."
            for nm in ("q_proj", "k_proj", "v_proj", "out_proj"):
                sd[p + f"self_attn.{nm}.weight"], sd[p + f"self_attn.{nm}.bias"] = n(E, E), zeros(E)
            sd[p + "self_attn_layer_norm.weight"], sd[p + "self_attn_layer_norm.bias"] = ones(E), zeros(E)
            sd[p + "fc1.weight"], sd[p + "fc1.bias"] = n(F, E), zeros(F)
            sd[p + "fc2.weight"], sd[p + "fc2.bias"] = n(E, F), zeros(E)
            sd[p + "final_layer_norm.weight"], sd[p + "final_layer_norm.bias"] = ones(E), zeros(E)
        sd[pre + "final_layer_norm.weight"], sd[pre + "final_layer_norm.bias"] = ones(E), zeros(E)
    return sd


def synthetic_weights_notice(model_version: str) -> None:
    if os.environ.get("EAVQA_REQUIRE_PRETRAINED", "0") == "1":
        raise FileNotFoundError(f"{model_version!r}: no local HF directory (EAVQA_MODEL_DIR) and EAVQA_REQUIRE_PRETRAINED=1 forbids "
                                "the seeded random-init stand-in")
    import warnings
    warnings.warn(f"{model_version!r} is not a local HF directory: using SEEDED RANDOM-INIT weights of that architecture (synthetic runs "
                  "only; set EAVQA_MODEL_DIR to a directory of HF checkpoints, or EAVQA_REQUIRE_PRETRAINED=1 to make this an error)",
                  RuntimeWarning, stacklevel=3)


def load_local_hf(path: str):
    with open(os.path.join(path, "config.json")) as f:
        cfg = json.load(f)
    st = os.path.join(path, "model.safetensors")
    if os.path.exists(st):
        from safetensors.torch import load_file
        return cfg, load_file(st)
    pt = os.path.join(path, "pytorch_model.bin")
    if os.path.exists(pt):
        return cfg, torch.load(pt, map_location="cpu", weights_only=True)
    raise FileNotFoundError(f"no model.safetensors / pytorch_model.bin under {path}")


class Fp8Weight:

    __slots__ = ("q", "scale", "shape")

    def __init__(self, q: Tensor, scale: float):
        self.q, self.scale, self.shape = q, float(scale), tuple(q.shape)

    @staticmethod
    def quantize(w: Tensor, device) -> "Fp8Weight":
        w = w.to(device=device, dtype=torch.float32)
        amax = float(w.abs().max().item())
        scale = amax / 448.0 if amax > 0 else 1.0
        q = (w / scale).to(torch.float8_e4m3fn).view(torch.uint8).contiguous()
        return Fp8Weight(q, scale)

    def t(self) -> "Fp8Weight":
        return Fp8Weight(self.q.T.contiguous(), self.scale)

    def dequantize(self) -> Tensor:
        return self.q.view(torch.float8_e4m3fn).float() * self.scale


def linear(a: Tensor, w, **kw) -> Tensor:
    if isinstance(w, Fp8Weight):
        aq, a_scale = a if isinstance(a, tuple) else ops.quantize_rows_fp8(a)
        return ops.gemm_fp8(aq, a_scale, w.q, w.scale, **kw)
    return ops.gemm(a, w, **kw)


class _Layer:
    __slots__ = ("ln1_g", "ln1_b", "w_qkv", "b_qkv", "w_o", "b_o", "ln2_g", "ln2_b", "w_fc1", "b_fc1", "w_fc2", "b_fc2",
                 "w_qkv_t", "w_o_t", "w_fc1_t", "w_fc2_t",
                 "w_qkv_f", "c_qkv", "d_qkv", "w_fc1_f", "c_fc1", "d_fc1")


class FrozenCausalLM:

    def __init__(self, cfg: LMConfig, state_dict: Dict[str, Tensor], dtype: torch.dtype = torch.bfloat16, device="cuda",
                 weight_format: str = "native"):
        self.cfg = cfg
        self.dtype = dtype
        self.device = torch.device(device)
        if weight_format not in ("native", "fp8"):
            raise ValueError("weight_format must be 'native' or 'fp8'")
        if weight_format == "fp8" and (dtype != torch.bfloat16 or cfg.n_embd % 128 or cfg.ffn % 128):
            raise ValueError("fp8 weights need bfloat16 activations and n_embd / ffn multiples of 128")
        self.weight_format = weight_format
        self._pack(state_dict)
        self._bwd_ready = False
        self.fold_layernorm = (dtype == torch.bfloat16 and weight_format == "native" and os.environ.get("EAVQA_LN_FOLD", "0") == "1")
        self._fold_ready = False
        self.fuse_quantizer = os.environ.get("EAVQA_FUSE_QUANT", "1") != "0"

    def _T(self, t: Tensor) -> Tensor:
        return t.to(device=self.device, dtype=self.dtype).contiguous()

    def _F(self, t: Tensor) -> Tensor:
        return t.to(device=self.device, dtype=torch.float32).contiguous()

    def _pack(self, sd: Dict[str, Tensor]) -> None:
        c = self.cfg
        self.layers = []
        if c.arch == "gpt2":
            self.wte = self._T(sd["transformer.wte.weight"])
            self.wpe = self._T(sd["transformer.wpe.weight"])
            for i in range(c.n_layer):
                p = f"transformer.h.{i}."
                L = _Layer()
                L.ln1_g, L.ln1_b = self._F(sd[p + "ln_1.weight"]), self._F(sd[p + "ln_1.bias"])
                L.w_qkv, L.b_qkv = self._T(sd[p + "attn.c_attn.weight"].T), self._F(sd[p + "attn.c_attn.bias"])
                L.w_o, L.b_o = self._T(sd[p + "attn.c_proj.weight"].T), self._F(sd[p + "attn.c_proj.bias"])
                L.ln2_g, L.ln2_b = self._F(sd[p + "ln_2.weight"]), self._F(sd[p + "ln_2.bias"])
                L.w_fc1, L.b_fc1 = self._T(sd[p + "mlp.c_fc.weight"].T), self._F(sd[p + "mlp.c_fc.bias"])
                L.w_fc2, L.b_fc2 = self._T(sd[p + "mlp.c_proj.weight"].T), self._F(sd[p + "mlp.c_proj.bias"])
                L.w_qkv_t = L.w_o_t = L.w_fc1_t = L.w_fc2_t = None
                self.layers.append(L)
            self.lnf_g, self.lnf_b = self._F(sd["transformer.ln_f.weight"]), self._F(sd["transformer.ln_f.bias"])
            head = sd.get("lm_head.weight")
        else:
            pre = "model.decoder."
            self.wte = self._T(sd[pre + "embed_tokens.weight"])
            self.wpe = self._T(sd[pre + "embed_positions.weight"])
            for i in range(c.n_layer):
                p = f"{pre}layers.{i}."
                L = _Layer()
                L.ln1_g, L.ln1_b = self._F(sd[p + "self_attn_layer_norm.weight"]), self._F(sd[p + "self_attn_layer_norm.bias"])
                L.w_qkv = self._T(torch.cat([sd[p + f"self_attn.{n}_proj.weight"] for n in "qkv"], dim=0))
                L.b_qkv = self._F(torch.cat([sd[p + f"self_attn.{n}_proj.bias"] for n in "qkv"], dim=0))
                L.w_o, L.b_o = self._T(sd[p + "self_attn.out_proj.weight"]), self._F(sd[p + "self_attn.out_proj.bias"])
                L.ln2_g, L.ln2_b = self._F(sd[p + "final_layer_norm.weight"]), self._F(sd[p + "final_layer_norm.bias"])
                L.w_fc1, L.b_fc1 = self._T(sd[p + "fc1.weight"]), self._F(sd[p + "fc1.bias"])
                L.w_fc2, L.b_fc2 = self._T(sd[p + "fc2.weight"]), self._F(sd[p + "fc2.bias"])
                L.w_qkv_t = L.w_o_t = L.w_fc1_t = L.w_fc2_t = None
                self.layers.append(L)
            self.lnf_g, self.lnf_b = self._F(sd[pre + "final_layer_norm.weight"]), self._F(sd[pre + "final_layer_norm.bias"])
            head = sd.get("lm_head.weight")
        self.head = self.wte if head is None or head.shape == self.wte.shape and _same(head, self.wte) else self._T(head)
        self.head_t = None
        self.head_q = None
        if self.weight_format == "fp8":
            for L in self.layers:
                for name in ("w_qkv", "w_o", "w_fc1", "w_fc2"):
                    setattr(L, name, Fp8Weight.quantize(getattr(L, name), self.device))
            self.head_q = Fp8Weight.quantize(self.head, self.device)

    @property
    def vocab(self) -> int:
        return self.wte.shape[0]

    @property
    def vpad(self) -> int:
        q = 128 if self.weight_format == "fp8" else 64
        return (self.vocab + q - 1) // q * q

    def _prepare_backward(self) -> None:
        if self._bwd_ready:
            return
        tr = (lambda w: w.t()) if self.weight_format == "fp8" else (lambda w: w.T.contiguous())
        for L in self.layers:
            L.w_qkv_t = tr(L.w_qkv)
            L.w_o_t = tr(L.w_o)
            L.w_fc1_t = tr(L.w_fc1)
            L.w_fc2_t = tr(L.w_fc2)
        V, E = self.head.shape
        if self.weight_format == "fp8":
            qt = torch.zeros((E, self.vpad), device=self.device, dtype=torch.uint8)
            qt[:, :V] = self.head_q.q.T
            self.head_t = Fp8Weight(qt, self.head_q.scale)
        else:
            self.head_t = torch.zeros((E, self.vpad), device=self.device, dtype=self.dtype)
            self.head_t[:, :V] = self.head.T
        self._bwd_ready = True

    def _prepare_fold(self) -> None:
        if self._fold_ready:
            return
        for L in self.layers:
            for w, b, g, be, nm in ((L.w_qkv, L.b_qkv, L.ln1_g, L.ln1_b, "qkv"), (L.w_fc1, L.b_fc1, L.ln2_g, L.ln2_b, "fc1")):
                w32 = w.float()
                wf = (w32 * g[None, :]).to(self.dtype).contiguous()
                setattr(L, f"w_{nm}_f", wf)
                setattr(L, f"c_{nm}", wf.float().sum(1).contiguous())
                setattr(L, f"d_{nm}", (w32 @ be + b).contiguous())
                del w32
        self._fold_ready = True

    def resize_token_embeddings(self, n: int) -> None:
        V, E = self.wte.shape
        if n == V:
            return
        tied = self.head is self.wte
        new = torch.empty((n, E), device=self.device, dtype=self.dtype)
        keep = min(n, V)
        new[:keep] = self.wte[:keep]
        if n > V:
            new[V:] = self.wte.float().mean(0).to(self.dtype)
        self.wte = new
        if tied:
            self.head = new
        else:
            h = torch.empty((n, E), device=self.device, dtype=self.dtype)
            h[:keep] = self.head[:keep]
            if n > V:
                h[V:] = self.head.float().mean(0).to(self.dtype)
            self.head = h
        self.cfg.vocab = n
        self._bwd_ready = False
        if self.weight_format == "fp8":
            self.head_q = Fp8Weight.quantize(self.head, self.device)

    def load_token_embeddings(self, weight: Tensor) -> None:
        if tuple(weight.shape) != tuple(self.wte.shape):
            raise ValueError(f"token embedding shape {tuple(weight.shape)} does not match {tuple(self.wte.shape)}")
        tied = self.head is self.wte
        self.wte = self._T(weight)
        if tied:
            self.head = self.wte
        self._bwd_ready = False
        if self.weight_format == "fp8":
            self.head_q = Fp8Weight.quantize(self.head, self.device)

    def forward(self, prefix_rows: Optional[Tensor], src: Tensor, pos: Tensor, mask: Tensor, B: int, S: int, *,
                labels: Optional[Tensor] = None, save: bool = False, logits: str = "none", pack: bool = False,
                lengths=None, n_scored: Optional[int] = None):
        c, T = self.cfg, self.dtype
        E, H, hd = c.n_embd, c.n_head, c.head_dim
        scale = hd ** -0.5
        cu = flat = row_labels = None
        M = B * S
        if pack:
            cu, src_r, pos_r, row_labels, flat = ops.build_row_plan(mask, labels, src, pos, True)
            M = int(sum(lengths)) if lengths is not None else int(cu[-1].item())
            src, pos, flat = src_r[:M], pos_r[:M], flat[:M]
            row_labels = row_labels[:M] if labels is not None else None
            attn_mask = None
        else:
            attn_mask = mask
        x = ops.embed_assemble(src, pos, self.wte, prefix_rows, self.wpe)
        tape = [] if save else None
        fold = self.fold_layernorm and M > 64
        if fold:
            self._prepare_fold()
        n_slots = (E + 63) // 64
        f32 = dict(device=self.device, dtype=torch.float32)
        fuse_q = self.weight_format == "fp8" and self.fuse_quantizer

        def ln(xx, g, b, stats):
            if fuse_q:
                r = ops.layernorm_fwd_fp8(xx, g, b, c.eps, save_stats=stats)
                return ((r[0], r[1]), r[2], r[3]) if stats else r
            return ops.layernorm_fwd(xx, g, b, c.eps, T, save_stats=stats)

        xT = st = None
        for li, L in enumerate(self.layers):
            if st is not None:
                mean1, rstd1 = (torch.empty(M, **f32), torch.empty(M, **f32)) if save else (None, None)
                qkv = ops.gemm(xT, L.w_qkv_f, bias=L.d_qkv, ln_stats=st, ln_c=L.c_qkv, ln_eps=c.eps, ln_save=(mean1, rstd1) if save else None)
            else:
                if save:
                    a, mean1, rstd1 = ln(x, L.ln1_g, L.ln1_b, True)
                else:
                    a = ln(x, L.ln1_g, L.ln1_b, False)
                qkv = linear(a, L.w_qkv, bias=L.b_qkv)
            q, k, v = qkv[:, :E], qkv[:, E:2 * E], qkv[:, 2 * E:]
            if save:
                ctx, lse = ops.attention_fwd(q, k, v, B, H, S, S, hd, key_mask=attn_mask, causal=True, scale=scale,
                                             save_lse=True, cu_seqlens=cu)
            else:
                ctx = ops.attention_fwd(q, k, v, B, H, S, S, hd, key_mask=attn_mask, causal=True, scale=scale, cu_seqlens=cu)
            if fold:
                x1T = torch.empty((M, E), device=self.device, dtype=T)
                st1 = torch.empty((M, n_slots, 2), **f32)
                x1 = ops.gemm(ctx, L.w_o, bias=L.b_o, residual=x, out_f32=True, copy_out=x1T, stats_out=st1)
                mean2, rstd2 = (torch.empty(M, **f32), torch.empty(M, **f32)) if save else (None, None)
                u = torch.empty((M, c.ffn), device=self.device, dtype=T) if save else None
                f = ops.gemm(x1T, L.w_fc1_f, bias=L.d_fc1, act=c.act, aux_out=u, ln_stats=st1, ln_c=L.c_fc1, ln_eps=c.eps,
                             ln_save=(mean2, rstd2) if save else None)
                if li + 1 < len(self.layers):
                    xT = torch.empty((M, E), device=self.device, dtype=T)
                    st = torch.empty((M, n_slots, 2), **f32)
                    x2 = ops.gemm(f, L.w_fc2, bias=L.b_fc2, residual=x1, out_f32=True, copy_out=xT, stats_out=st)
                else:
                    x2 = ops.gemm(f, L.w_fc2, bias=L.b_fc2, residual=x1, out_f32=True)
            else:
                x1 = linear(ctx, L.w_o, bias=L.b_o, residual=x, out_f32=True)
                if save:
                    a2, mean2, rstd2 = ln(x1, L.ln2_g, L.ln2_b, True)
                    u = torch.empty((M, c.ffn), device=self.device, dtype=T)
                    f = linear(a2, L.w_fc1, bias=L.b_fc1, act=c.act, aux_out=u)
                else:
                    a2 = ln(x1, L.ln2_g, L.ln2_b, False)
                    f = linear(a2, L.w_fc1, bias=L.b_fc1, act=c.act)
                x2 = linear(f, L.w_fc2, bias=L.b_fc2, residual=x1, out_f32=True)
            if save:
                tape.append((x, mean1, rstd1, qkv, ctx, lse, x1, mean2, rstd2, u))
            x = x2
        out = {"rows": M, "flat_index": flat}
        if logits == "last" and labels is None and not pack:
            xl = x.view(B, S, E)[:, -1]
            hf = ops.layernorm_fwd(xl, self.lnf_g, self.lnf_b, c.eps, T)
            out["logits"] = self._head(hf)
            return out
        if save:
            hf, meanf, rstdf = ops.layernorm_fwd(x, self.lnf_g, self.lnf_b, c.eps, T, save_stats=True)
        else:
            hf = ops.layernorm_fwd(x, self.lnf_g, self.lnf_b, c.eps, T)
        out["hidden"] = hf
        if labels is not None or logits == "all":
            sel = sel_count = None
            if pack and labels is not None and n_scored is not None and logits != "all" and 0 < n_scored < M:
                sel, ce_labels, sel_count = ops.select_rows(row_labels, int(n_scored))
                lg = self._head(ops.gather_rows(hf, sel))
            else:
                lg = self._head(hf)
                ce_labels = row_labels if pack else labels
            out["logits"], out["sel"] = lg, sel
            if labels is not None:
                loss, count, row_lse = ops.ce_fwd(lg, ce_labels, self.vocab)
                if sel_count is not None:
                    ops.guard_count(sel_count, int(n_scored), loss)
                out["loss"], out["count"] = loss, count
                if save:
                    out["tape"] = dict(layers=tape, x_last=x, meanf=meanf, rstdf=rstdf, logits=lg, labels=ce_labels, sel=sel,
                                       row_lse=row_lse, count=count, src=src, mask=attn_mask, cu=cu, B=B, S=S, M=M)
        return out

    def _head(self, hf: Tensor) -> Tensor:
        lg = torch.empty((hf.shape[0], self.vpad), device=self.device, dtype=torch.float32)
        if self.head_q is not None:
            linear(hf, self.head_q, out=lg[:, :self.vocab])
            return lg
        if hf.shape[0] <= 64 and hf.dtype == torch.bfloat16 and self.vocab % 4 == 0 and self.cfg.n_embd % 32 == 0:
            ops.splitk_finish(ops.gemm_splitk(hf, self.head[:self.vocab]), [lg[:, :self.vocab]])
        else:
            ops.gemm(hf, self.head, out=lg[:, :self.vocab])
        return lg

    def backward(self, tape: dict, gloss: Tensor, n_prefix_rows: int) -> Tensor:
        self._prepare_backward()
        c, T = self.cfg, self.dtype
        E, H, hd = c.n_embd, c.n_head, c.head_dim
        B, S, M = tape["B"], tape["S"], tape["M"]
        scale = hd ** -0.5
        mask, cu = tape["mask"], tape["cu"]
        lowp = T != torch.float32

        dlog = ops.ce_bwd(tape["logits"], tape["labels"], self.vocab, tape["row_lse"], tape["count"], gloss, T, self.vpad)
        dhf = linear(dlog, self.head_t)
        if tape.get("sel") is not None:
            dhf = ops.scatter_rows(dhf, tape["sel"], M)
        fuse_q = self.weight_format == "fp8" and self.fuse_quantizer
        if fuse_q:
            dxq = (torch.empty((M, E), device=self.device, dtype=torch.uint8), torch.empty(M, device=self.device, dtype=torch.float32))
            dxT = dxq

            def ln_bwd(xx, dy, g, mean, rstd, **kw):
                return ops.layernorm_bwd_fp8(xx, dy, g, mean, rstd, dxq[0], dxq[1], **kw)
        else:
            dxT = torch.empty((M, E), device=self.device, dtype=T) if lowp else None

            def ln_bwd(xx, dy, g, mean, rstd, **kw):
                return ops.layernorm_bwd(xx, dy, g, mean, rstd, lowp_out=dxT, **kw)
        dx = ln_bwd(tape["x_last"], dhf, self.lnf_g, tape["meanf"], tape["rstdf"])
        for L, (x, mean1, rstd1, qkv, ctx, lse, x1, mean2, rstd2, u) in zip(reversed(self.layers), reversed(tape["layers"])):
            du = linear(dxT if lowp else dx, L.w_fc2_t, act=c.act, aux_in=u)
            da2 = linear(du, L.w_fc1_t)
            dx1 = ln_bwd(x1, da2, L.ln2_g, mean2, rstd2, dres=dx, out=dx)
            dctx = linear(dxT if lowp else dx1, L.w_o_t)
            dqkv = torch.empty_like(qkv)
            q, k, v = qkv[:, :E], qkv[:, E:2 * E], qkv[:, 2 * E:]
            ops.attention_bwd(q, k, v, ctx, dctx, lse, B, H, S, S, hd, key_mask=mask, causal=True, scale=scale,
                              dq=dqkv[:, :E], dk=dqkv[:, E:2 * E], dv=dqkv[:, 2 * E:], cu_seqlens=cu)
            da = linear(dqkv, L.w_qkv_t)
            dx = ln_bwd(x, da, L.ln1_g, mean1, rstd1, dres=dx1, out=dx1)
        return ops.embed_assemble_bwd(tape["src"], dx, n_prefix_rows, T)


def _same(a: Tensor, b: Tensor) -> bool:
    try:
        return a.data_ptr() == b.data_ptr() or bool(torch.equal(a.to(b.device, b.dtype), b))
    except Exception:
        return False
```

### explicit-alignment-for-vqa-tasks_amd/ops.py

```python
from __future__ import annotations

import ctypes as C
from typing import Optional, Tuple

import torch

from . import _lib
from ._lib import ACT, BF16, F32, call

Tensor = torch.Tensor


F16 = 2


def dtype_id(dt: torch.dtype, stream: bool = False) -> int:
    if dt == torch.float32:
        return F32
    if dt == torch.bfloat16:
        return BF16
    if stream and dt == torch.float16:
        return F16
    raise _lib.EavqaError(f"unsupported storage dtype {dt}")


def _stream() -> int:
    return torch._C._cuda_getCurrentRawStream(torch._C._cuda_getDevice())


class KernelSelect:
    gemm = 0
    attention = 0
    decode_route = 0


def _p(t: Optional[Tensor]) -> Optional[int]:
    return None if t is None else t.data_ptr()


def _dev(t: Tensor) -> None:
    if not t.is_cuda:
        raise _lib.EavqaError("eavqa ops run on the GPU only (no CPU fallback): got a CPU tensor")


def _ld(t: Tensor) -> int:
    if t.stride(-1) != 1 and t.shape[-1] != 1:
        raise _lib.EavqaError("last dimension must be contiguous")
    return t.stride(-2) if t.dim() >= 2 else t.shape[-1]


def gemm(a: Tensor, b: Tensor, *, a_kc: bool = True, b_kc: bool = True, bias: Optional[Tensor] = None,
         act: str = "none", aux_in: Optional[Tensor] = None, aux_out: Optional[Tensor] = None,
         residual: Optional[Tensor] = None, out: Optional[Tensor] = None, out_f32: bool = False,
         alpha: float = 1.0, copy_out: Optional[Tensor] = None, stats_out: Optional[Tensor] = None, ln_stats: Optional[Tensor] = None,
         ln_c: Optional[Tensor] = None, ln_eps: float = 1e-5, ln_save: Optional[Tuple[Tensor, Tensor]] = None) -> Tensor:
    _dev(a)
    M, K = (a.shape if a_kc else (a.shape[1], a.shape[0]))
    N, Kb = (b.shape if b_kc else (b.shape[1], b.shape[0]))
    if K != Kb:
        raise _lib.EavqaError(f"gemm inner dims differ: {K} vs {Kb}")
    if a.dtype != b.dtype:
        raise _lib.EavqaError("gemm operands must share a dtype")
    dt = dtype_id(a.dtype)
    half = torch.float16
    if out is None:
        out = torch.empty((M, N), device=a.device, dtype=torch.float32 if out_f32 else a.dtype)
    elif out.dtype != torch.float32 and out.dtype != a.dtype and not (out.dtype == half and a.dtype == torch.bfloat16):
        raise _lib.EavqaError("gemm out dtype must be float32, the operand dtype or (bf16 operands) float16")
    out_f32 = out.dtype == torch.float32
    aux = aux_in if aux_in is not None else aux_out
    flags = int(out_f32)
    if residual is not None and residual.dtype != torch.float32:
        if residual.dtype != a.dtype and not (residual.dtype == half and a.dtype == torch.bfloat16):
            raise _lib.EavqaError("gemm residual must be float32, the operand dtype or (bf16 operands) float16")
        flags |= 2
    stream_half = (out.dtype == half) or (residual is not None and residual.dtype == half)
    if stream_half:
        if (out.dtype not in (half, torch.float32)) or (residual is not None and residual.dtype not in (half, torch.float32)):
            raise _lib.EavqaError("gemm: a float16 stream needs float16 (or float32) for both the residual and the output")
        flags |= 4
    args = (dt, int(a_kc), int(b_kc), M, N, K, _p(a), _ld(a), _p(b), _ld(b), _p(out), _ld(out),
            flags, float(alpha), _p(bias), ACT[act], _p(aux_in), _p(aux_out), _ld(aux) if aux is not None else 0,
            _p(residual), _ld(residual) if residual is not None else 0, _stream())
    if copy_out is not None or stats_out is not None or ln_stats is not None:
        g = _lib.GemmLn()
        if copy_out is not None:
            if copy_out.dtype != a.dtype or tuple(copy_out.shape) != (M, N):
                raise _lib.EavqaError("gemm copy_out must be [M, N] in the operand dtype")
            g.copy_out, g.ld_copy = _p(copy_out), _ld(copy_out)
        if stats_out is not None:
            if stats_out.dtype != torch.float32 or stats_out.dim() != 3 or stats_out.shape[0] != M or stats_out.shape[2] != 2 or not stats_out.is_contiguous():
                raise _lib.EavqaError("gemm stats_out must be a contiguous float32 [M, slots, 2]")
            g.stats_out, g.stats_ld = _p(stats_out), stats_out.shape[1]
        if ln_stats is not None:
            if ln_stats.dtype != torch.float32 or ln_stats.dim() != 3 or ln_stats.shape[0] != M or ln_stats.shape[2] != 2 or not ln_stats.is_contiguous():
                raise _lib.EavqaError("gemm ln_stats must be a contiguous float32 [M, slots, 2]")
            if ln_c is None or ln_c.dtype != torch.float32 or ln_c.numel() != N:
                raise _lib.EavqaError("gemm ln_c must be float32 [N]")
            g.ln_stats, g.ln_parts, g.ln_ld, g.ln_cols = _p(ln_stats), ln_stats.shape[1], ln_stats.shape[1], K
            g.ln_c, g.ln_eps = _p(ln_c), float(ln_eps)
            if ln_save is not None:
                g.mean_out, g.rstd_out = _p(ln_save[0]), _p(ln_save[1])
        if KernelSelect.gemm:
            call("eavqa_gemm_ln_ex", *args[:-1], C.byref(g), args[-1], KernelSelect.gemm)
        else:
            call("eavqa_gemm_ln", *args[:-1], C.byref(g), args[-1])
    elif KernelSelect.gemm:
        call("eavqa_gemm_ex", *args, KernelSelect.gemm)
    else:
        call("eavqa_gemm", *args)
    return out


def quantize_rows_fp8(x: Tensor):
    _dev(x)
    rows, cols = x.shape
    q = torch.empty((rows, cols), device=x.device, dtype=torch.uint8)
    sc = torch.empty(rows, device=x.device, dtype=torch.float32)
    call("eavqa_quantize_rows_fp8", dtype_id(x.dtype), rows, cols, _p(x), _ld(x), _p(q), _ld(q), _p(sc), _stream())
    return q, sc


def gemm_fp8(a_q: Tensor, a_scale: Tensor, b_q: Tensor, b_scale: float, *, bias: Optional[Tensor] = None, act: str = "none",
             aux_in: Optional[Tensor] = None, aux_out: Optional[Tensor] = None, residual: Optional[Tensor] = None,
             out: Optional[Tensor] = None, out_f32: bool = False, alpha: float = 1.0, tile: int = 0) -> Tensor:
    _dev(a_q)
    M, K = a_q.shape
    N = b_q.shape[0]
    if b_q.shape[1] != K:
        raise _lib.EavqaError(f"gemm_fp8 inner dims differ: {K} vs {b_q.shape[1]}")
    if out is None:
        out = torch.empty((M, N), device=a_q.device, dtype=torch.float32 if out_f32 else torch.bfloat16)
    aux = aux_in if aux_in is not None else aux_out
    call("eavqa_gemm_fp8", M, N, K, _p(a_q), _ld(a_q), _p(a_scale), _p(b_q), _ld(b_q), float(b_scale), _p(out), _ld(out),
         int(out.dtype == torch.float32), float(alpha), _p(bias), ACT[act], _p(aux_in), _p(aux_out), _ld(aux) if aux is not None else 0,
         _p(residual), _ld(residual) if residual is not None else 0, _stream(), int(tile))
    return out


def layernorm_fwd(x: Tensor, gamma: Optional[Tensor], beta: Optional[Tensor], eps: float, out_dtype: torch.dtype,
                  save_stats: bool = False, out: Optional[Tensor] = None):
    _dev(x)
    rows, cols = x.shape
    y = out if out is not None else torch.empty((rows, cols), device=x.device, dtype=out_dtype)
    mean = rstd = None
    if save_stats:
        mean = torch.empty(rows, device=x.device, dtype=torch.float32)
        rstd = torch.empty(rows, device=x.device, dtype=torch.float32)
    x_kind = {torch.float32: 1, torch.bfloat16: 2, torch.float16: 3}.get(x.dtype)
    if x_kind is None:
        raise _lib.EavqaError(f"unsupported layernorm input dtype {x.dtype}")
    call("eavqa_layernorm_fwd", dtype_id(out_dtype, stream=True), x_kind, rows, cols, _p(x), _ld(x),
         _p(gamma), _p(beta), float(eps), _p(y), _ld(y), _p(mean), _p(rstd), _stream())
    return (y, mean, rstd) if save_stats else y


def layernorm_fwd_fp8(x: Tensor, gamma: Optional[Tensor], beta: Optional[Tensor], eps: float, save_stats: bool = False):
    _dev(x)
    rows, cols = x.shape
    q = torch.empty((rows, cols), device=x.device, dtype=torch.uint8)
    sc = torch.empty(rows, device=x.device, dtype=torch.float32)
    mean = rstd = None
    if save_stats:
        mean = torch.empty(rows, device=x.device, dtype=torch.float32)
        rstd = torch.empty(rows, device=x.device, dtype=torch.float32)
    x_kind = {torch.float32: 1, torch.bfloat16: 2, torch.float16: 3}.get(x.dtype)
    if x_kind is None:
        raise _lib.EavqaError(f"unsupported layernorm input dtype {x.dtype}")
    call("eavqa_layernorm_fwd_fp8", x_kind, rows, cols, _p(x), _ld(x), _p(gamma), _p(beta), float(eps), _p(q), _ld(q), _p(sc), _p(mean), _p(rstd),
         _stream())
    return (q, sc, mean, rstd) if save_stats else (q, sc)


def layernorm_bwd_fp8(x: Tensor, dy: Tensor, gamma: Optional[Tensor], mean: Tensor, rstd: Tensor, q_out: Tensor, scale_out: Tensor,
                      dres: Optional[Tensor] = None, out: Optional[Tensor] = None) -> Tensor:
    _dev(x)
    rows, cols = x.shape
    if dy.dtype != torch.bfloat16:
        raise _lib.EavqaError("layernorm_bwd_fp8: dy must be bfloat16")
    dx = out if out is not None else torch.empty((rows, cols), device=x.device, dtype=torch.float32)
    if dres is not None and _ld(dres) != _ld(dx):
        raise _lib.EavqaError("dres must share dx's leading dimension")
    call("eavqa_layernorm_bwd_fp8", int(x.dtype == torch.float32), rows, cols, _p(x), _ld(x), _p(dy), _ld(dy), _p(gamma), _p(mean), _p(rstd),
         _p(dres), _p(dx), _ld(dx), _p(q_out), _ld(q_out), _p(scale_out), _stream())
    return dx


def layernorm_bwd(x: Tensor, dy: Tensor, gamma: Optional[Tensor], mean: Tensor, rstd: Tensor,
                  dres: Optional[Tensor] = None, dgamma: Optional[Tensor] = None, dbeta: Optional[Tensor] = None,
                  out: Optional[Tensor] = None, lowp_out: Optional[Tensor] = None) -> Tensor:
    _dev(x)
    rows, cols = x.shape
    dx = out if out is not None else torch.empty((rows, cols), device=x.device, dtype=torch.float32)
    if dres is not None and _ld(dres) != _ld(dx):
        raise _lib.EavqaError("dres must share dx's leading dimension")
    call("eavqa_layernorm_bwd", dtype_id(dy.dtype), int(x.dtype == torch.float32), rows, cols, _p(x), _ld(x), _p(dy), _ld(dy),
         _p(gamma), _p(mean), _p(rstd), _p(dres), _p(dx), _ld(dx), _p(dgamma), _p(dbeta), _p(lowp_out),
         _ld(lowp_out) if lowp_out is not None else 0, _stream())
    return dx


def attention_fwd(q: Tensor, k: Tensor, v: Tensor, B: int, H: int, Sq: int, Sk: int, hd: int, *,
                  key_mask: Optional[Tensor] = None, causal: bool = False, scale: float = 1.0, save_lse: bool = False,
                  q_batch_rows: int = 0, kv_batch_rows: int = 0, ld_mask: int = 0, out: Optional[Tensor] = None,
                  cu_seqlens: Optional[Tensor] = None):
    _dev(q)
    o = out if out is not None else torch.empty((q.shape[0] if cu_seqlens is not None else B * Sq, H * hd), device=q.device, dtype=q.dtype)
    lse = torch.empty((B, H, Sq), device=q.device, dtype=torch.float32) if save_lse else None
    args = (dtype_id(q.dtype), B, H, Sq, Sk, hd, _p(q), _ld(q), _p(k), _ld(k), _p(v), _ld(v), _p(o), _ld(o),
            q_batch_rows, kv_batch_rows, _p(key_mask), ld_mask, _p(cu_seqlens), int(causal), float(scale), _p(lse), _stream())
    if KernelSelect.attention:
        call("eavqa_attention_fwd_ex", *args, KernelSelect.attention)
    else:
        call("eavqa_attention_fwd", *args)
    return (o, lse) if save_lse else o


def attention_decode(q: Tensor, k_cache: Tensor, v_cache: Tensor, k_new: Tensor, v_new: Tensor, B: int, H: int, Sk: int, hd: int, *,
                     kv_batch_rows: int, key_mask: Optional[Tensor] = None, ld_mask: int = 0, scale: float = 1.0,
                     out: Optional[Tensor] = None) -> Tensor:
    _dev(q)
    o = out if out is not None else torch.empty((B, H * hd), device=q.device, dtype=q.dtype)
    call("eavqa_attention_decode", dtype_id(q.dtype), B, H, Sk, hd, _p(q), _ld(q), _p(k_cache), _ld(k_cache), _p(v_cache), _ld(v_cache),
         kv_batch_rows, _p(k_new), _p(v_new), _ld(k_new), _p(o), _ld(o), _p(key_mask), ld_mask, float(scale), _stream())
    return o


def attention_decode_splitk(part: Tensor, bias: Optional[Tensor], k_cache: Tensor, v_cache: Tensor, B: int, H: int, Sk: int, hd: int, *,
                            kv_batch_rows: int, key_mask: Optional[Tensor] = None, ld_mask: int = 0, scale: float = 1.0,
                            out: Optional[Tensor] = None) -> Tensor:
    _dev(part)
    o = out if out is not None else torch.empty((B, H * hd), device=part.device, dtype=k_cache.dtype)
    call("eavqa_attention_decode_splitk", dtype_id(k_cache.dtype), B, H, Sk, hd, _p(part), part.shape[0], _p(bias), _p(k_cache), _ld(k_cache),
         _p(v_cache), _ld(v_cache), kv_batch_rows, _p(o), _ld(o), _p(key_mask), ld_mask, float(scale), _stream())
    return o


def attention_bwd(q, k, v, o, d_o, lse, B, H, Sq, Sk, hd, *, key_mask=None, causal=False, scale=1.0,
                  dq=None, dk=None, dv=None, cu_seqlens=None):
    _dev(q)
    nq = q.shape[0] if cu_seqlens is not None else B * Sq
    nk = k.shape[0] if cu_seqlens is not None else B * Sk
    dq = dq if dq is not None else torch.empty((nq, H * hd), device=q.device, dtype=q.dtype)
    dk = dk if dk is not None else torch.empty((nk, H * hd), device=q.device, dtype=q.dtype)
    dv = dv if dv is not None else torch.empty((nk, H * hd), device=q.device, dtype=q.dtype)
    delta = torch.empty((B, H, Sq), device=q.device, dtype=torch.float32)
    args = (dtype_id(q.dtype), B, H, Sq, Sk, hd, _p(q), _ld(q), _p(k), _ld(k), _p(v), _ld(v), _p(o), _ld(o),
            _p(d_o), _ld(d_o), _p(dq), _ld(dq), _p(dk), _ld(dk), _p(dv), _ld(dv), _p(key_mask), _p(cu_seqlens), int(causal),
            float(scale), _p(lse), _p(delta), _stream())
    if KernelSelect.attention:
        call("eavqa_attention_bwd_ex", *args, KernelSelect.attention)
    else:
        call("eavqa_attention_bwd", *args)
    return dq, dk, dv


def build_prefix_rows(tokens: Tensor, question_mask: Tensor, L: int, pos_mode: int, prefix_row_stride: Optional[int] = None,
                      prefix_row_offset: int = 0):
    _dev(tokens)
    B, T = tokens.shape
    tokens = tokens.contiguous()
    qm = question_mask.to(torch.int64).contiguous()
    S = L + T
    src = torch.empty((B, S), device=tokens.device, dtype=torch.int32)
    msk = torch.empty_like(src)
    pos = torch.empty_like(src)
    call("eavqa_build_prefix_rows", B, L, T, _p(tokens), _p(qm), pos_mode, L if prefix_row_stride is None else prefix_row_stride,
         prefix_row_offset, _p(src), _p(msk), _p(pos), _stream())
    return src, msk, pos


def build_fewshot_rows(tokens: Tensor, question_mask: Tensor, L: int, n_img: int, special_token_id: int, pos_mode: int):
    _dev(tokens)
    B, T = tokens.shape
    tokens = tokens.contiguous()
    qm = question_mask.to(torch.int64).contiguous()
    T_out = T + (L - 1) * n_img
    src = torch.empty((B, T_out), device=tokens.device, dtype=torch.int32)
    msk = torch.empty_like(src)
    pos = torch.empty_like(src)
    status = torch.empty(B, device=tokens.device, dtype=torch.int32)
    call("eavqa_build_fewshot_rows", B, T, L, n_img, int(special_token_id), _p(tokens), _p(qm), pos_mode, _p(src), _p(msk),
         _p(pos), _p(status), _stream())
    return src, msk, pos, status


def embed_assemble(src: Tensor, pos: Optional[Tensor], wte: Tensor, prefix_rows: Optional[Tensor], wpe: Optional[Tensor],
                   out: Optional[Tensor] = None) -> Tensor:
    _dev(src)
    rows = src.numel()
    E = wte.shape[1]
    x = out if out is not None else torch.empty((rows, E), device=src.device, dtype=torch.float32)
    call("eavqa_embed_assemble", dtype_id(wte.dtype), rows, E, _p(src), _p(pos), _p(wte), _ld(wte), _p(prefix_rows),
         _ld(prefix_rows) if prefix_rows is not None else 0, _p(wpe), _ld(wpe) if wpe is not None else 0, _p(x), _ld(x), _stream())
    return x


def embed_assemble_bwd(src: Tensor, dx: Tensor, n_prefix_rows: int, dtype: torch.dtype) -> Tensor:
    rows, E = dx.shape
    d = torch.zeros((n_prefix_rows, E), device=dx.device, dtype=dtype)
    call("eavqa_embed_assemble_bwd", dtype_id(dtype), rows, E, _p(src), _p(dx), _ld(dx), _p(d), _ld(d), _stream())
    return d


def build_labels(input_ids: Tensor, L: int, pad_token_id: int, bos_token_id: int = -1, mode: int = 0) -> Tensor:
    _dev(input_ids)
    B, T = input_ids.shape
    ids = input_ids.contiguous()
    out = torch.empty((B, L + T), device=ids.device, dtype=torch.int64)
    call("eavqa_build_labels", mode, B, T, L, _p(ids), int(pad_token_id), int(bos_token_id), _p(out), _stream())
    return out


def build_row_plan(mask: Tensor, labels: Optional[Tensor], src: Tensor, pos: Tensor, pack: bool):
    _dev(mask)
    B, S = mask.shape
    dev = mask.device
    cu = torch.empty(B + 1, device=dev, dtype=torch.int32)
    src_r = torch.empty(B * S, device=dev, dtype=torch.int32)
    pos_r = torch.empty(B * S, device=dev, dtype=torch.int32)
    flat = torch.empty(B * S, device=dev, dtype=torch.int32)
    lab = torch.empty(B * S, device=dev, dtype=torch.int64)
    call("eavqa_build_row_plan", B, S, int(pack), _p(mask), _p(labels), _p(src), _p(pos), _p(cu), _p(src_r), _p(pos_r), _p(lab),
         _p(flat), _stream())
    return cu, src_r, pos_r, lab, flat


def _ce_dims(labels: Tensor):
    if labels.dim() == 2:
        return labels.shape[0], labels.shape[1], labels.shape[0] * labels.shape[1]
    return labels.shape[0], 0, labels.shape[0]


def ce_fwd(logits: Tensor, labels: Tensor, V: int):
    _dev(logits)
    B, S, rows = _ce_dims(labels)
    row_loss = torch.empty(rows, device=logits.device, dtype=torch.float32)
    row_lse = torch.empty(rows, device=logits.device, dtype=torch.float32)
    loss = torch.empty(1, device=logits.device, dtype=torch.float32)
    count = torch.empty(1, device=logits.device, dtype=torch.float32)
    call("eavqa_ce_fwd", B, S, V, _p(logits), _ld(logits), _p(labels), _p(row_loss), _p(row_lse), _p(loss), _p(count), _stream())
    return loss, count, row_lse


def guard_count(count: Tensor, capacity: int, loss: Tensor) -> None:
    call("eavqa_guard_count", _p(count), int(capacity), _p(loss), _stream())


def ce_bwd(logits: Tensor, labels: Tensor, V: int, row_lse: Tensor, count: Tensor, gscale: Tensor, dtype: torch.dtype,
           ldd: int) -> Tensor:
    B, S, rows = _ce_dims(labels)
    d = torch.empty((rows, ldd), device=logits.device, dtype=dtype)
    call("eavqa_ce_bwd", dtype_id(dtype), B, S, V, _p(logits), _ld(logits), _p(labels), _p(row_lse), _p(count), _p(gscale),
         _p(d), ldd, _stream())
    return d


def greedy_pick(logits: Tensor, V: int, pad_token_id: int, eos_token_id: Optional[int], raw: Tensor, emitted_col: Tensor,
                unfinished: Tensor, logprob: Optional[Tensor] = None, any_unfinished: Optional[Tensor] = None) -> None:
    B = logits.shape[0]
    call("eavqa_greedy_pick", B, V, _p(logits), _ld(logits), int(pad_token_id if pad_token_id is not None else 0),
         int(eos_token_id) if eos_token_id is not None else -1, _p(raw), _p(emitted_col), emitted_col.stride(0),
         _p(unfinished), _p(logprob), _p(any_unfinished), _stream())


def adamw(param: Tensor, grad: Tensor, m: Tensor, v: Tensor, step: int, lr: float, beta1: float = 0.9, beta2: float = 0.999,
          eps: float = 1e-8, weight_decay: float = 0.01, grad_scale: float = 1.0, shadow: Optional[Tensor] = None) -> None:
    _dev(param)
    call("eavqa_adamw", param.numel(), _p(param), _p(grad), _p(m), _p(v), int(step), float(lr), float(beta1), float(beta2),
         float(eps), float(weight_decay), float(grad_scale), dtype_id(shadow.dtype) if shadow is not None else 0, _p(shadow), _stream())


def patchify(pixels: Tensor, ps: int, dtype: torch.dtype, ldp: int) -> Tensor:
    _dev(pixels)
    B, C3, img, _ = pixels.shape
    g = img // ps
    pixels = pixels.contiguous().float()
    out = torch.empty((B * g * g, ldp), device=pixels.device, dtype=dtype)
    call("eavqa_patchify", dtype_id(dtype), B, img, ps, _p(pixels), _p(out), ldp, _stream())
    return out


def vit_assemble(patch_embed: Tensor, cls: Tensor, pos: Tensor, B: int, n_patch: int) -> Tensor:
    W = patch_embed.shape[1]
# ... 249 lines not shown
```

### include/eavqa.h

```cpp
#ifndef EAVQA_H
#define EAVQA_H

#include <stdint.h>

#ifdef __cplusplus
extern "C" {
#endif
#pragma GCC visibility push(default)

#define EAVQA_ABI_VERSION 1

enum { EAVQA_F32 = 0, EAVQA_BF16 = 1,
       EAVQA_F16 = 2 };

enum { EAVQA_GEMM_OUT_F32 = 1, EAVQA_GEMM_RESIDUAL_LOWP = 2, EAVQA_GEMM_STREAM_F16 = 4 };
enum { EAVQA_ACT_NONE = 0, EAVQA_ACT_TANH = 1, EAVQA_ACT_RELU = 2, EAVQA_ACT_GELU_NEW = 3, EAVQA_ACT_QUICK_GELU = 4 };

enum {
    EAVQA_OK = 0,
    EAVQA_E_ARG = -1,
    EAVQA_E_ALIGN = -2,
    EAVQA_E_SHAPE = -3,
    EAVQA_E_DTYPE = -4,
    EAVQA_E_LAUNCH = -5,
    EAVQA_E_ARCH = -6
};

int eavqa_abi_version(void);
const char* eavqa_strerror(int code);
int eavqa_check_device(void);

int eavqa_gemm(int dtype, int a_kc, int b_kc, int M, int N, int K,
               const void* A, int64_t lda, const void* B, int64_t ldb,
               void* C, int64_t ldc, int out_flags, float alpha,
               const float* bias, int act,
               const void* aux_in, void* aux_out, int64_t ld_aux,
               const void* residual, int64_t ldr, void* stream);

typedef struct {
    void* copy_out; int64_t ld_copy;
    float* stats_out; int32_t stats_ld;
    const float* ln_stats; int32_t ln_parts; int32_t ln_ld; int32_t ln_cols;
    const float* ln_c; float ln_eps;
    float* mean_out; float* rstd_out;
} eavqa_gemm_ln_t;
int eavqa_gemm_ln(int dtype, int a_kc, int b_kc, int M, int N, int K,
                  const void* A, int64_t lda, const void* B, int64_t ldb,
                  void* C, int64_t ldc, int out_flags, float alpha,
                  const float* bias, int act,
                  const void* aux_in, void* aux_out, int64_t ld_aux,
                  const void* residual, int64_t ldr, const eavqa_gemm_ln_t* ln, void* stream);

int eavqa_layernorm_fwd(int dtype, int x_kind, int rows, int cols, const void* x, int64_t ldx,
                        const float* gamma, const float* beta, float eps,
                        void* y, int64_t ldy, float* mean, float* rstd, void* stream);
int eavqa_layernorm_bwd(int dtype, int x_f32, int rows, int cols, const void* x, int64_t ldx,
                        const void* dy, int64_t lddy, const float* gamma,
                        const float* mean, const float* rstd,
                        const float* dres, float* dx, int64_t lddx,
                        float* dgamma, float* dbeta, void* dx_lowp, int64_t ld_lowp, void* stream);
int eavqa_layernorm_fwd_fp8(int x_kind, int rows, int cols, const void* x, int64_t ldx, const float* gamma, const float* beta,
                            float eps, void* yq, int64_t ldq, float* row_scale, float* mean, float* rstd, void* stream);
int eavqa_layernorm_bwd_fp8(int x_f32, int rows, int cols, const void* x, int64_t ldx, const void* dy, int64_t lddy,
                            const float* gamma, const float* mean, const float* rstd, const float* dres, float* dx, int64_t lddx,
                            void* dxq, int64_t ldq, float* row_scale, void* stream);


int eavqa_attention_fwd(int dtype, int B, int H, int Sq, int Sk, int hd,
                        const void* q, int64_t ldq, const void* k, int64_t ldk,
                        const void* v, int64_t ldv, void* o, int64_t ldo,
                        int64_t q_batch_rows, int64_t kv_batch_rows,
                        const int32_t* key_mask, int64_t ld_mask, const int32_t* cu_seqlens, int causal, float scale,
                        float* lse, void* stream);
int eavqa_attention_decode(int dtype, int B, int H, int Sk, int hd, const void* q, int64_t ldq, void* k_cache, int64_t ldk,
                           void* v_cache, int64_t ldv, int64_t kv_batch_rows, const void* k_new, const void* v_new, int64_t ld_new,
                           void* o, int64_t ldo, const int32_t* key_mask, int64_t ld_mask, float scale, void* stream);
int eavqa_attention_decode_splitk(int dtype, int B, int H, int Sk, int hd, const float* qkv_partials, int ks, const float* qkv_bias,
                                  void* k_cache, int64_t ldk, void* v_cache, int64_t ldv, int64_t kv_batch_rows, void* o, int64_t ldo,
                                  const int32_t* key_mask, int64_t ld_mask, float scale, void* stream);
int eavqa_attention_bwd(int dtype, int B, int H, int Sq, int Sk, int hd,
                        const void* q, int64_t ldq, const void* k, int64_t ldk,
                        const void* v, int64_t ldv, const void* o, int64_t ldo,
                        const void* d_o, int64_t lddo,
                        void* dq, int64_t lddq, void* dk, int64_t lddk, void* dv, int64_t lddv,
                        const int32_t* key_mask, const int32_t* cu_seqlens, int causal, float scale,
                        const float* lse, float* delta, void* stream);

int eavqa_build_prefix_rows(int B, int L, int T, const int64_t* tokens, const int64_t* question_mask,
                            int pos_mode, int prefix_row_stride, int prefix_row_offset,
                            int32_t* src, int32_t* mask_out, int32_t* pos, void* stream);
int eavqa_build_fewshot_rows(int B, int T, int L, int n_img, int64_t special_token_id,
                             const int64_t* tokens, const int64_t* question_mask, int pos_mode,
                             int32_t* src, int32_t* mask_out, int32_t* pos, int32_t* status, void* stream);
int eavqa_build_row_plan(int B, int S, int pack, const int32_t* mask, const int64_t* labels, const int32_t* src,
                         const int32_t* pos, int32_t* cu_seqlens, int32_t* src_rows, int32_t* pos_rows,
                         int64_t* row_labels, int32_t* flat_index, void* stream);
int eavqa_copy_rows(int dtype, int B, int S, int cols, const void* src, int64_t lds, int64_t src_batch_rows,
                    void* dst, int64_t ldd, int64_t dst_batch_rows, int64_t dst_row0, void* stream);
int eavqa_select_rows(int M, const int64_t* row_labels, int capacity, int32_t* sel_idx, int64_t* sel_labels, int32_t* count,
                      void* stream);
int eavqa_move_rows(int dtype, int scatter, int n, int cols, const void* src, int64_t ld_src, const int32_t* idx, void* dst,
                    int64_t ld_dst, void* stream);
int eavqa_transpose(int dtype, int rows, int cols, const void* src, int64_t ld_src, void* dst, int64_t ld_dst, void* stream);
int eavqa_colsum(int dtype, int rows, int cols, const void* x, int64_t ldx, float* out, int accumulate, void* stream);
int eavqa_embed_assemble(int dtype, int rows, int E, const int32_t* src, const int32_t* pos,
                         const void* wte, int64_t ld_wte, const void* prefix_rows, int64_t ld_prefix,
                         const void* wpe, int64_t ld_wpe, float* x, int64_t ldx, void* stream);
int eavqa_embed_assemble_bwd(int dtype, int rows, int E, const int32_t* src, const float* dx, int64_t lddx,
                             void* dprefix, int64_t ld_dprefix, void* stream);

int eavqa_build_labels(int mode, int B, int T, int L, const int64_t* input_ids, int64_t pad_token_id,
                       int64_t bos_token_id, int64_t* labels_out, void* stream);

int eavqa_ce_fwd(int B, int S, int V, const float* logits, int64_t ld, const int64_t* labels,
                 float* row_loss, float* row_lse, float* loss, float* count, void* stream);
int eavqa_guard_count(const int32_t* count, int capacity, float* loss, void* stream);
int eavqa_ce_bwd(int dtype, int B, int S, int V, const float* logits, int64_t ld, const int64_t* labels,
                 const float* row_lse, const float* count, const float* gscale,
                 void* dlogits, int64_t ldd, void* stream);
int eavqa_greedy_pick(int B, int V, const float* logits, int64_t ld, int64_t pad_token_id, int64_t eos_token_id,
                      int32_t* raw, int64_t* emitted, int64_t ld_emitted, int32_t* unfinished, float* logprob,
                      int32_t* any_unfinished, void* stream);

int eavqa_adamw(int64_t n, float* param, const float* grad, float* m, float* v, int step,
                float lr, float beta1, float beta2, float eps, float weight_decay, float grad_scale,
                int shadow_dtype, void* shadow, void* stream);

int eavqa_patchify(int dtype, int B, int img, int ps, const float* pixels, void* patches, int64_t ldp, void* stream);
int eavqa_vit_assemble(int dtype, int B, int n_patch, int W, const void* patch_embed, int64_t ldpe,
                       const float* cls, const float* pos, float* x, int64_t ldx, void* stream);

typedef struct {
    const float* ln1_g; const float* ln1_b;
    const void* w_qkv; const float* b_qkv;
    const void* w_o; const float* b_o;
    const float* ln2_g; const float* ln2_b;
    const void* w_fc1; const float* b_fc1;
    const void* w_fc2; const float* b_fc2;
    void* k_cache; void* v_cache;
} eavqa_lm_layer_t;
int64_t eavqa_lm_block_workspace_bytes(int dtype, int rows, int E, int F);
int eavqa_lm_block_forward(int dtype, int n_layer, const eavqa_lm_layer_t* layers, int E, int H, int F, int act, float eps,
                           int B, int Sq, int row0, int S_max, float* x, const int32_t* key_mask, int64_t ld_mask,
                           void* workspace, int64_t workspace_bytes, void* stream);

typedef struct { float s_qkv, s_o, s_fc1, s_fc2; } eavqa_lm_layer_scales_t;
int64_t eavqa_lm_block_fp8_workspace_bytes(int rows, int E, int F);
int eavqa_lm_block_forward_fp8(int n_layer, const eavqa_lm_layer_t* layers, const eavqa_lm_layer_scales_t* scales, int E, int H, int F, int act,
                               float eps, int B, int Sq, int row0, int S_max, float* x, const int32_t* key_mask, int64_t ld_mask,
                               void* workspace, int64_t workspace_bytes, void* stream);

typedef struct {
    const float* ln_sa; const void* w_qkv; const void* w_o;
    const float* ln_ca; const void* w_q_ca; const void* w_o_ca;
    const float* ln_ff; const void* w_i; const void* w_o_ff;
    void* k_cache; void* v_cache;
    const void* cross_kv;
} eavqa_t5_dec_layer_t;
int64_t eavqa_t5_decoder_step_workspace_bytes(int dtype, int B, int E, int inner, int F, int gated);
int eavqa_t5_decoder_step(int dtype, int n_layer, const eavqa_t5_dec_layer_t* layers, const float* ln_final, int E, int inner, int H,
                          int F, int gated, int act, float eps, int B, int t, int t_max, int S, float* x, void* out,
                          const int32_t* enc_mask, int64_t ld_mask, const float* rel_bias, int64_t rel_ld, int rel_zero,
                          void* workspace, int64_t workspace_bytes, void* stream);

int eavqa_gemm_splitk_plan(int M, int N, int K);
int eavqa_gemm_splitk(int dtype, int M, int N, int K, const void* A, int64_t lda, const void* B, int64_t ldb,
                      float* partials, int ks, void* stream);
int eavqa_splitk_finish(int dtype, int M, int N, const float* partials, int ks, const float* bias, int act,
                        const float* residual, int64_t ld_residual, int out_f32, int n_seg,
                        void* out0, int64_t ld0, void* out1, int64_t ld1, void* out2, int64_t ld2, void* stream);
int eavqa_layernorm_splitk(int dtype, int rows, int cols, const float* x_in, int64_t ldx, const float* partials, int ks,
                           const float* bias, float* x_out, int64_t ld_out, const float* gamma, const float* beta,
                           float eps, void* y, int64_t ldy, void* stream);

int eavqa_gemm_fp8_splitk_plan(int M, int N, int K);
int eavqa_gemm_fp8_splitk(int M, int N, int K, const void* A, int64_t lda, const float* a_row_scale, const void* B, int64_t ldb,
                          float b_scale, float* partials, int ks, void* stream);
int eavqa_layernorm_splitk_fp8(int rows, int cols, const float* x_in, int64_t ldx, const float* partials, int ks, const float* bias,
                               float* x_out, int64_t ld_out, const float* gamma, const float* beta, float eps, void* yq, int64_t ldq,
                               float* row_scale, void* stream);

int eavqa_rmsnorm_splitk(int dtype, int rows, int cols, const float* x_in, int64_t ldx, const float* partials, int ks,
                         float* x_out, int64_t ld_out, const float* gamma, float eps, void* y, int64_t ldy, void* stream);
int eavqa_splitk_finish_gated(int dtype, int M, int F, const float* partials, int ks, int act, void* out, int64_t ld, void* stream);
int eavqa_attention_decode_splitk_rel(int dtype, int B, int H, int Sk, int hd, const float* partials, int ks, int part_cols,
                                      void* k, int64_t ldk, void* v, int64_t ldv, int64_t kv_batch_rows, void* o, int64_t ldo,
                                      const int32_t* key_mask, int64_t ld_mask, float scale, const float* rel_bias, int64_t rel_ld,
                                      int rel_zero, void* stream);

typedef struct {
    int M, N, K;
    const void* A; int64_t lda; int a_kind;
    const float* gamma; const float* beta; float eps;
    const float* stats_in; int n_stats_in; int stats_in_cols;
    const void* B; int64_t ldb; int gated_rows;
    const float* bias; int act;
    const float* residual; int64_t ld_residual;
    int out_f32; int n_seg; void* out[3]; int64_t ld_out[3];
    float* stats_out;
} eavqa_decode_gemm_t;
int eavqa_gemm_decode_cols(int M, int N, int K, int a_kind, int gated);
int eavqa_gemm_decode(const eavqa_decode_gemm_t* args, void* stream);

int eavqa_l2_normalize_rows(int rows, int cols, float* x, int64_t ld, void* stream);
int eavqa_topk_rows(int rows, int cols, const float* scores, int64_t ld, int k, float* out_val, int64_t* out_idx, void* stream);

int eavqa_quantize_rows_fp8(int dtype, int rows, int cols, const void* x, int64_t ldx, void* out, int64_t ld_out,
                            float* row_scale, void* stream);
int eavqa_gemm_fp8(int M, int N, int K, const void* A, int64_t lda, const float* a_row_scale, const void* B, int64_t ldb,
                   float b_scale, void* C, int64_t ldc, int out_f32, float alpha, const float* bias, int act,
                   const void* aux_in, void* aux_out, int64_t ld_aux, const float* residual, int64_t ldr, void* stream, int tile);

int eavqa_rmsnorm_fwd(int dtype, int x_kind, int rows, int cols, const void* x, int64_t ldx, const float* gamma, float eps,
                      void* y, int64_t ldy, float* rstd, void* stream);
int eavqa_rmsnorm_bwd(int dtype, int x_kind, int rows, int cols, const void* x, int64_t ldx, const void* dy, int64_t lddy,
                      const float* gamma, const float* rstd, const float* dres, float* dx, int64_t lddx, void* dx_lowp,
                      int64_t ld_lowp, void* stream);
int eavqa_gated_act_fwd(int dtype, int rows, int F, int act, const void* u, int64_t ldu, void* h, int64_t ldh, void* stream);
int eavqa_gated_act_bwd(int dtype, int rows, int F, int act, const void* u, int64_t ldu, const void* dh, int64_t lddh,
                        void* du, int64_t lddu, void* stream);
int eavqa_attention_fwd_rel(int dtype, int B, int H, int Sq, int Sk, int hd, const void* q, int64_t ldq, const void* k, int64_t ldk,
                            const void* v, int64_t ldv, void* o, int64_t ldo, int64_t q_batch_rows, int64_t kv_batch_rows,
                            const int32_t* key_mask, int64_t ld_mask, int causal, float scale, const float* rel_bias,
                            int64_t rel_ld, int rel_zero, float* lse, void* stream);
int eavqa_attention_bwd_rel(int dtype, int B, int H, int Sq, int Sk, int hd, const void* q, int64_t ldq, const void* k, int64_t ldk,
                            const void* v, int64_t ldv, const void* o, int64_t ldo, const void* d_o, int64_t lddo,
                            void* dq, int64_t lddq, void* dk, int64_t lddk, void* dv, int64_t lddv,
                            const int32_t* key_mask, int causal, float scale, const float* rel_bias, int64_t rel_ld,
                            int rel_zero, const float* lse, float* delta, void* stream);

int eavqa_cast_rows(int dtype, int rows, int64_t cols, const float* x, int64_t ldx, void* y, int64_t ldy, void* stream);

#pragma GCC visibility pop
#ifdef __cplusplus
}
#endif
#endif
```

Measured before the change: 4710 samples/s.

## Pre-pack frozen weights into swizzled K64 tiles for direct LDS loads

Measured after the change: 4688 samples/s. About the same (-0.5%).

```diff
diff --git a/explicit-alignment-for-vqa-tasks_amd/_lib.py b/explicit-alignment-for-vqa-tasks_amd/_lib.py
--- a/explicit-alignment-for-vqa-tasks_amd/_lib.py
+++ b/explicit-alignment-for-vqa-tasks_amd/_lib.py
@@ -30,6 +30,9 @@
     "eavqa_build_row_plan": [i32, i32, i32, ptr, ptr, ptr, ptr, ptr, ptr, ptr, ptr, ptr, ptr],
     "eavqa_copy_rows": [i32, i32, i32, i32, ptr, i64, i64, ptr, i64, i64, i64, ptr],
     "eavqa_transpose": [i32, i32, i32, ptr, i64, ptr, i64, ptr],
+    "eavqa_pack_k64": [i32, i32, i32, ptr, i64, i64, ptr, ptr],
+    "eavqa_pack_k64_offset": [i32, i32, i32, i32],
+    "eavqa_gemm_reads_packed": [i32, i32, i32],
     "eavqa_select_rows": [i32, ptr, i32, ptr, ptr, ptr, ptr],
     "eavqa_move_rows": [i32, i32, i32, i32, ptr, i64, ptr, ptr, i64, ptr],
     "eavqa_l2_normalize_rows": [i32, i32, ptr, i64, ptr],
@@ -112,7 +115,7 @@
 SIGNATURES["eavqa_gemm_decode_ex"] = SIGNATURES["eavqa_gemm_decode"] + [i32]
 SIGNATURES["eavqa_t5_decoder_step_ex"] = SIGNATURES["eavqa_t5_decoder_step"] + [i32]
 
-_RESTYPES = {"eavqa_strerror": C.c_char_p, "eavqa_lm_block_workspace_bytes": C.c_int64, "eavqa_lm_block_fp8_workspace_bytes": C.c_int64, "eavqa_t5_decoder_step_workspace_bytes": C.c_int64}
+_RESTYPES = {"eavqa_strerror": C.c_char_p, "eavqa_pack_k64_offset": C.c_int64, "eavqa_lm_block_workspace_bytes": C.c_int64, "eavqa_lm_block_fp8_workspace_bytes": C.c_int64, "eavqa_t5_decoder_step_workspace_bytes": C.c_int64}
 
 _lib = None
 
diff --git a/explicit-alignment-for-vqa-tasks_amd/build.py b/explicit-alignment-for-vqa-tasks_amd/build.py
--- a/explicit-alignment-for-vqa-tasks_amd/build.py
+++ b/explicit-alignment-for-vqa-tasks_amd/build.py
@@ -16,7 +16,7 @@
 LIB = os.path.join(CSRC, "libeavqa_hip.so")
 EXPORTS = os.path.join(CSRC, "exports.map")
 
-HIP_SOURCES = ["gemm.hip", "norm.hip", "attention.hip", "seq.hip", "loss.hip", "optim.hip", "decode.hip", "decode_direct.hip", "retrieval.hip"]
+HIP_SOURCES = ["gemm.hip", "pack.hip", "norm.hip", "attention.hip", "seq.hip", "loss.hip", "optim.hip", "decode.hip", "decode_direct.hip", "retrieval.hip"]
 CPP_SOURCES = ["api.cpp", "lm_block.cpp", "t5_block.cpp"]
 ARCH = "gfx950"
 
diff --git a/explicit-alignment-for-vqa-tasks_amd/csrc/gemm.hip b/explicit-alignment-for-vqa-tasks_amd/csrc/gemm.hip
--- a/explicit-alignment-for-vqa-tasks_amd/csrc/gemm.hip
+++ b/explicit-alignment-for-vqa-tasks_amd/csrc/gemm.hip
@@ -22,6 +22,7 @@
     const float* bias; const void* aux_in; void* aux_out; const void* residual;
     const float* row_scale;
     int M, N, K;
+    int b_pack;
     int64_t lda, ldb, ldc, ld_aux, ldr;
     int act, out_f32, res_lowp;
     int out_f16;
@@ -1240,8 +1241,15 @@
               void* C, int64_t ldc, int out_flags, float alpha,
               const float* bias, int act,
               const void* aux_in, void* aux_out, int64_t ld_aux,
-              const void* residual, int64_t ldr, const eavqa_gemm_ln_t* ln, void* stream, int knobs) {
+              const void* residual, int64_t ldr, const eavqa_gemm_ln_t* ln, void* stream, int knobs, int* route = nullptr) {
     const Knobs kn(knobs);
+    const int b_pack = b_kc == EAVQA_B_K64_PACKED;
+    if (b_pack) {
+        if (dtype != EAVQA_BF16 || !a_kc) return EAVQA_E_SHAPE;
+        if (K <= 0 || (K % 64) != 0 || (ldb % 8) != 0) return EAVQA_E_ALIGN;
+        if (ldb < N || ldb - N >= 8) return EAVQA_E_ARG;
+        b_kc = 1;
+    }
     const bool ln_consumer = ln && ln->ln_stats;
     if (ln) {
         if (ln->copy_out && ln->ld_copy < N) return EAVQA_E_ARG;
@@ -1262,15 +1270,15 @@
     const int vec = dtype == EAVQA_BF16 ? 8 : 4;
     const int a_contig = a_kc ? K : M, b_contig = b_kc ? K : N;
     if (a_contig % vec || b_contig % vec) return EAVQA_E_SHAPE;
-    if (lda % vec || ldb % vec) return EAVQA_E_ALIGN;
+    if (lda % vec || (!b_pack && ldb % vec)) return EAVQA_E_ALIGN;
     if (!eavqa_aligned16(A) || !eavqa_aligned16(B)) return EAVQA_E_ALIGN;
-    if (lda < a_contig || ldb < b_contig || ldc < N) return EAVQA_E_ARG;
+    if (lda < a_contig || (!b_pack && ldb < b_contig) || ldc < N) return EAVQA_E_ARG;
     if ((aux_in || aux_out) && ld_aux < N) return EAVQA_E_ARG;
     if (residual && ldr < N) return EAVQA_E_ARG;
 
     GemmParams p;
     p.A = A; p.B = B; p.C = C; p.bias = bias; p.aux_in = aux_in; p.aux_out = aux_out; p.residual = residual; p.row_scale = nullptr; p.ablate = kn.ablate;
-    p.M = M; p.N = N; p.K = K; p.lda = lda; p.ldb = ldb; p.ldc = ldc; p.ld_aux = ld_aux; p.ldr = ldr;
+    p.M = M; p.N = N; p.K = K; p.b_pack = b_pack; p.lda = lda; p.ldb = ldb; p.ldc = ldc; p.ld_aux = ld_aux; p.ldr = ldr;
     p.act = act; p.out_f32 = out_f32; p.res_lowp = res_lowp; p.out_f16 = stream_f16 && !out_f32; p.alpha = alpha;
     p.group_n = kn.group_n == 0 ? BIG_GROUP_N : kn.group_n - 1;
     p.tiles_m = (M + BM - 1) / BM;
@@ -1295,7 +1303,8 @@
     if (dtype == EAVQA_BF16) {
         if (a_kc && b_kc && (K % 64) == 0 && kn.k64_mode >= 2 && kn.k64_mode < 2 + N_K64) return K64_SHAPES[kn.k64_mode - 2].launch(p, s);
         const bool few_columns = kn.k64_mode == 0 && kn.shape_mode == 0 && kn.big_mode == 0 && N <= 4096;
-        if (!ln && a_kc && b_kc && !kn.disable_fast && M <= 64 && (K % 32) == 0 && N >= 64 && (kn.k64_mode == 1 || (K % 64) != 0 || few_columns)) return launch_skinny(p, s);
+        if (!ln && !b_pack && a_kc && b_kc && !kn.disable_fast && M <= 64 && (K % 32) == 0 && N >= 64 && (kn.k64_mode == 1 || (K % 64) != 0 || few_columns))
+            return route ? EAVQA_OK : launch_skinny(p, s);
         const int big_rem = (a_kc && b_kc && kn.big_mode != 1 && !kn.no_row_split) ? big_split_rows(M, N) : 0;
         const float big_split_ns = big_rem ? 12000.f : 0.f;
         auto run_big = [&](const GemmParams& pp) -> int {
@@ -1319,7 +1328,7 @@
         int bgx, bgy;
         const int big_rounds = (big_grid((M - big_rem + GBM - 1) / GBM, (N + GBN - 1) / GBN, bgx, bgy) + 31) / 32;
         const bool many_big_tiles = big_rounds >= 4 || (big_rounds >= 2 && (M + GBM - 1) / GBM > 96);
-        if (a_kc && b_kc && !kn.disable_fast && (K % 64) == 0 && kn.k64_mode != 1 && kn.shape_mode == 0 && kn.big_mode == 0 && !many_big_tiles) {
+        if (a_kc && b_kc && !kn.disable_fast && (K % 64) == 0 && kn.k64_mode != 1 && kn.shape_mode == 0 && kn.big_mode == 0 && (!many_big_tiles || b_pack)) {
             int pick = K64_AUTO[0];
             float best_loop = 0.f;
             float best = k64_cost(p, K64_SHAPES[pick], &best_loop);
@@ -1330,9 +1339,13 @@
             }
             best += 0.35f * best_loop;
             const float big_cost = float(big_rounds) * (float(K / 64) * (big_rounds == 1 ? 1380.f : 1530.f) + 9000.f) + 3000.f + big_split_ns;
-            if (M > 64 && big_cost < best) return run_big(p);
+            const bool to_big = M > 64 && big_cost < best && !b_pack;
+            if (route) { *route = !to_big; return EAVQA_OK; }
+            if (to_big) return run_big(p);
             return K64_SHAPES[pick].launch(p, s);
         }
+        if (b_pack) return EAVQA_E_SHAPE;
+        if (route) return EAVQA_OK;
         if (a_kc && b_kc && !kn.disable_fast && (K % FBK) == 0 && !ln) {
             if (kn.shape_mode >= 2 && kn.shape_mode < 7) return SHAPES[kn.shape_mode - 2].launch(p, s);
             const bool big_ok = (K % GBK) == 0 && kn.big_mode != 1;
@@ -1359,6 +1372,7 @@
         if (!a_kc && b_kc) return launch(gemm_bf16_kernel<false, true>, p, s);
         return launch(gemm_bf16_kernel<false, false>, p, s);
     }
+    if (route) return EAVQA_OK;
     if (a_kc && b_kc) return launch(gemm_f32_kernel<true, true>, p, s);
     if (a_kc && !b_kc) return launch(gemm_f32_kernel<true, false>, p, s);
     if (!a_kc && b_kc) return launch(gemm_f32_kernel<false, true>, p, s);
@@ -1374,6 +1388,15 @@
                              const void* residual, int64_t ldr, void* stream, int knobs) {
     return gemm_impl(dtype, a_kc, b_kc, M, N, K, A, lda, B, ldb, C, ldc, out_flags, alpha, bias, act, aux_in, aux_out, ld_aux, residual, ldr,
                      nullptr, stream, knobs);
+}
+
+extern "C" int eavqa_gemm_reads_packed(int M, int N, int K) {
+    if (M <= 0 || N <= 0 || K <= 0 || (K % 64) != 0) return 0;
+    int route = 0;
+    void* const dummy = reinterpret_cast<void*>(uintptr_t(16));
+    const int rc = gemm_impl(EAVQA_BF16, 1, 1, M, N, K, dummy, K, dummy, K, dummy, N, 0, 1.f, nullptr, EAVQA_ACT_NONE, nullptr, nullptr, 0,
+                             nullptr, 0, nullptr, nullptr, 0, &route);
+    return rc == EAVQA_OK ? route : 0;
 }
 
 extern "C" int eavqa_gemm_ln_ex(int dtype, int a_kc, int b_kc, int M, int N, int K,
@@ -1445,7 +1468,7 @@
     if ((aux_in || aux_out) && ld_aux < N) return EAVQA_E_ARG;
     if (residual && ldr < N) return EAVQA_E_ARG;
     GemmParams p;
-    p.A = A; p.B = B; p.C = C; p.bias = bias; p.aux_in = aux_in; p.aux_out = aux_out; p.residual = residual; p.row_scale = a_row_scale; p.ablate = 0;
+    p.A = A; p.B = B; p.C = C; p.bias = bias; p.aux_in = aux_in; p.aux_out = aux_out; p.residual = residual; p.row_scale = a_row_scale; p.ablate = 0; p.b_pack = 0;
     p.M = M; p.N = N; p.K = K; p.lda = lda; p.ldb = ldb; p.ldc = ldc; p.ld_aux = ld_aux; p.ldr = ldr;
     p.act = act; p.out_f32 = out_f32; p.res_lowp = 0; p.out_f16 = 0; p.alpha = alpha * b_scale;
     p.group_n = 0;
diff --git a/explicit-alignment-for-vqa-tasks_amd/csrc/gemm_k64.hip b/explicit-alignment-for-vqa-tasks_amd/csrc/gemm_k64.hip
--- a/explicit-alignment-for-vqa-tasks_amd/csrc/gemm_k64.hip
+++ b/explicit-alignment-for-vqa-tasks_amd/csrc/gemm_k64.hip
@@ -23,18 +23,26 @@
 
 template <class G>
 __device__ __forceinline__ void k64s_loader_role(const char* A, const char* B, int64_t lda_bytes, int64_t ldb_bytes, int M, int N, int m0,
-                                                 int n0, int nk, char* smem, int lw, int lane) {
+                                                 int n0, int nk, char* smem, int lw, int lane, int b_groups = 0, int64_t b_gpitch = 0) {
     constexpr int NST = G::NST;
     const bool hi = lw < G::N_HI;
     const char* src[G::P_HI];
-    int dst[G::P_HI];
+    int dst[G::P_HI], kstep[G::P_HI];
 #pragma unroll
     for (int i = 0; i < G::P_HI; ++i) {
         const int piece = min(lw + G::LW * i, G::PT - 1);
         const int row = piece * 8 + (lane >> 3), slot = lane & 7;
         const int kc = (slot ^ (lane >> 3)) * 16;
-        src[i] = row < G::TBM ? A + (int64_t)min(m0 + row, M - 1) * lda_bytes + kc
-                              : B + (int64_t)min(n0 + row - G::TBM, N - 1) * ldb_bytes + kc;
+        const bool is_a = piece < G::TBM / 8;
+        if (is_a || b_groups == 0) {
+            src[i] = is_a ? A + (int64_t)min(m0 + row, M - 1) * lda_bytes + kc
+                          : B + (int64_t)min(n0 + row - G::TBM, N - 1) * ldb_bytes + kc;
+            kstep[i] = 128;
+        } else {
+            const int g = min((n0 >> 3) + piece - G::TBM / 8, b_groups - 1);
+            src[i] = B + (int64_t)g * b_gpitch + lane * 16;
+            kstep[i] = 1024;
+        }
         dst[i] = piece * 1024;
     }
     auto issue = [&](int kt, int stage) {
@@ -42,7 +50,7 @@
 #pragma unroll
         for (int i = 0; i < G::P_HI; ++i)
             if (i < G::P_LO || hi)
-                __builtin_amdgcn_global_load_lds((const __attribute__((address_space(1))) void*)(src[i] + (int64_t)kt * 128),
+                __builtin_amdgcn_global_load_lds((const __attribute__((address_space(1))) void*)(src[i] + (int64_t)kt * kstep[i]),
                                                  (__attribute__((address_space(3))) void*)(st + dst[i]), 16, 0, 0);
     };
     auto wait_tiles = [&](int tiles) {
@@ -128,8 +136,9 @@
     float2* rowstat = reinterpret_cast<float2*>(smem + G::RING);
 
     if (wave >= G::NC) {
+        const int b_groups = p.b_pack ? int(p.ldb >> 3) : 0;
         k64s_loader_role<G>(reinterpret_cast<const char*>(p.A), reinterpret_cast<const char*>(p.B), p.lda * 2, p.ldb * 2, p.M, p.N, m0, n0, nk,
-                            smem, wave - G::NC, lane);
+                            smem, wave - G::NC, lane, b_groups, int64_t(p.K >> 6) * 1024);
     } else {
         const int frow = lane & 15, fk = lane >> 4;
         const int sw0 = ((fk ^ (frow & 7)) << 4);
diff --git a/explicit-alignment-for-vqa-tasks_amd/csrc/pack.hip b/explicit-alignment-for-vqa-tasks_amd/csrc/pack.hip
--- /dev/null
+++ b/explicit-alignment-for-vqa-tasks_amd/csrc/pack.hip
@@ -0,0 +1,49 @@
+#include "common.h"
+
+namespace {
+
+__global__ __launch_bounds__(256) void pack_k64_kernel(int R, int K, const uint16_t* __restrict__ src, int64_t rs, int64_t cs, char* __restrict__ dst) {
+    __shared__ uint16_t tile[64][66];
+    const int kb = blockIdx.x, g0 = blockIdx.y * 8, t = threadIdx.x;
+    const int row0 = g0 * 8, col0 = kb * 64;
+    const bool along_k = cs <= rs;
+#pragma unroll 4
+    for (int i = 0; i < 16; ++i) {
+        const int idx = i * 256 + t;
+        const int r = along_k ? idx >> 6 : idx & 63, k = along_k ? idx & 63 : idx >> 6;
+        tile[r][k] = row0 + r < R ? src[(int64_t)(row0 + r) * rs + (int64_t)(col0 + k) * cs] : uint16_t(0);
+    }
+    __syncthreads();
+    const int groups = (R + 7) >> 3, kblocks = K >> 6;
+#pragma unroll
+    for (int i = 0; i < 2; ++i) {
+        const int j = i * 256 + t, gl = j >> 6, l = j & 63;
+        if (g0 + gl >= groups) continue;
+        const int r = l >> 3, c = (l & 7) ^ r;
+        const uint16_t* e = &tile[gl * 8 + r][c * 8];
+        uint4 v;
+        v.x = e[0] | (uint32_t(e[1]) << 16); v.y = e[2] | (uint32_t(e[3]) << 16);
+        v.z = e[4] | (uint32_t(e[5]) << 16); v.w = e[6] | (uint32_t(e[7]) << 16);
+        *reinterpret_cast<uint4*>(dst + ((int64_t)(g0 + gl) * kblocks + kb) * 1024 + l * 16) = v;
+    }
+}
+
+}
+
+extern "C" int64_t eavqa_pack_k64_offset(int rows, int cols, int row, int col) {
+    if (rows <= 0 || cols <= 0 || (cols % 64) != 0 || row < 0 || col < 0 || row >= ((rows + 7) & ~7) || col >= cols) return -1;
+    const int64_t block = (int64_t)(row >> 3) * (cols >> 6) + (col >> 6);
+    return block * 1024 + (row & 7) * 128 + ((((col >> 3) & 7) ^ (row & 7)) * 16) + (col & 7) * 2;
+}
+
+extern "C" int eavqa_pack_k64(int dtype, int rows, int cols, const void* src, int64_t row_stride, int64_t col_stride, void* dst, void* stream) {
+    if (rows <= 0 || cols <= 0 || !src || !dst || row_stride <= 0 || col_stride <= 0) return EAVQA_E_ARG;
+    if (dtype != EAVQA_BF16) return EAVQA_E_DTYPE;
+    if (cols % 64) return EAVQA_E_SHAPE;
+    if (!eavqa_aligned16(dst) || (reinterpret_cast<uintptr_t>(src) & 1u)) return EAVQA_E_ALIGN;
+    const int groups = (rows + 7) / 8;
+    hipLaunchKernelGGL(pack_k64_kernel, dim3(cols / 64, (groups + 7) / 8), dim3(256), 0, reinterpret_cast<hipStream_t>(stream), rows, cols,
+                       static_cast<const uint16_t*>(src), row_stride, col_stride, static_cast<char*>(dst));
+    EAVQA_LAUNCH_CHECK();
+    return EAVQA_OK;
+}
diff --git a/explicit-alignment-for-vqa-tasks_amd/models/clip_vit.py b/explicit-alignment-for-vqa-tasks_amd/models/clip_vit.py
--- a/explicit-alignment-for-vqa-tasks_amd/models/clip_vit.py
+++ b/explicit-alignment-for-vqa-tasks_amd/models/clip_vit.py
@@ -1,5 +1,6 @@
 from __future__ import annotations
 
+import os
 from dataclasses import dataclass
 from typing import Dict
 
@@ -102,6 +103,19 @@
                 w_fc2=T(state_dict[q + "mlp.fc2.weight"]), b_fc2=F(state_dict[q + "mlp.fc2.bias"]),
             ))
 
+        self.packed_weights = dtype == torch.bfloat16 and W % 64 == 0 and os.environ.get("EAVQA_PACKED_WEIGHTS", "1") != "0"
+        self._packed_ready = False
+
+    _WEIGHTS = ("w_qkv", "w_o", "w_fc1", "w_fc2")
+
+    def _prepare_packed(self, M: int) -> bool:
+        if not self._packed_ready and any(ops.gemm_reads_packed(M, *self.layers[0][n].shape) for n in self._WEIGHTS):
+            for L in self.layers:
+                for n in self._WEIGHTS:
+                    L[n + "_p"] = ops.pack_k64(L[n])
+            self._packed_ready = True
+        return self._packed_ready
+
     @torch.no_grad()
     def encode_image(self, pixels: Tensor) -> Tensor:
         c, T = self.cfg, self.dtype
@@ -116,14 +130,16 @@
         ST = self.stream_dtype
         x = ops.layernorm_fwd(x, self.pre_g, self.pre_b, c.eps, ST)
         x1 = torch.empty_like(x)
+        packed = self.packed_weights and B * N > 64 and self._prepare_packed(B * N)
+        gemm = ops.gemm_frozen if packed else (lambda a_, w_, wp_, **kw: ops.gemm(a_, w_, **kw))
         for L in self.layers:
             a = ops.layernorm_fwd(x, L["ln1_g"], L["ln1_b"], c.eps, T)
-            qkv = ops.gemm(a, L["w_qkv"], bias=L["b_qkv"])
+            qkv = gemm(a, L["w_qkv"], L.get("w_qkv_p"), bias=L["b_qkv"])
             ctx = ops.attention_fwd(qkv[:, :W], qkv[:, W:2 * W], qkv[:, 2 * W:], B, H, N, N, hd, causal=False, scale=hd ** -0.5)
-            ops.gemm(ctx, L["w_o"], bias=L["b_o"], residual=x, out=x1)
+            gemm(ctx, L["w_o"], L.get("w_o_p"), bias=L["b_o"], residual=x, out=x1)
             a2 = ops.layernorm_fwd(x1, L["ln2_g"], L["ln2_b"], c.eps, T)
-            f = ops.gemm(a2, L["w_fc1"], bias=L["b_fc1"], act=c.act)
-            ops.gemm(f, L["w_fc2"], bias=L["b_fc2"], residual=x1, out=x)
+            f = gemm(a2, L["w_fc1"], L.get("w_fc1_p"), bias=L["b_fc1"], act=c.act)
+            gemm(f, L["w_fc2"], L.get("w_fc2_p"), bias=L["b_fc2"], residual=x1, out=x)
         pooled = ops.layernorm_fwd(x.view(B, N, W)[:, 0], self.post_g, self.post_b, c.eps, T)
         return ops.gemm(pooled, self.w_proj, out_f32=True)
 
diff --git a/explicit-alignment-for-vqa-tasks_amd/models/lm.py b/explicit-alignment-for-vqa-tasks_amd/models/lm.py
--- a/explicit-alignment-for-vqa-tasks_amd/models/lm.py
+++ b/explicit-alignment-for-vqa-tasks_amd/models/lm.py
@@ -158,6 +158,7 @@
 class _Layer:
     __slots__ = ("ln1_g", "ln1_b", "w_qkv", "b_qkv", "w_o", "b_o", "ln2_g", "ln2_b", "w_fc1", "b_fc1", "w_fc2", "b_fc2",
                  "w_qkv_t", "w_o_t", "w_fc1_t", "w_fc2_t",
+                 "w_qkv_p", "w_o_p", "w_fc1_p", "w_fc2_p",
                  "w_qkv_f", "c_qkv", "d_qkv", "w_fc1_f", "c_fc1", "d_fc1")
 
 
@@ -175,6 +176,9 @@
         self.weight_format = weight_format
         self._pack(state_dict)
         self._bwd_ready = False
+        self.packed_weights = (dtype == torch.bfloat16 and weight_format == "native" and cfg.n_embd % 64 == 0 and cfg.ffn % 64 == 0
+                               and os.environ.get("EAVQA_PACKED_WEIGHTS", "1") != "0")
+        self._fwd_packed_ready = False
         self.fold_layernorm = (dtype == torch.bfloat16 and weight_format == "native" and os.environ.get("EAVQA_LN_FOLD", "0") == "1")
         self._fold_ready = False
         self.fuse_quantizer = os.environ.get("EAVQA_FUSE_QUANT", "1") != "0"
@@ -201,6 +205,7 @@
                 L.w_fc1, L.b_fc1 = self._T(sd[p + "mlp.c_fc.weight"].T), self._F(sd[p + "mlp.c_fc.bias"])
                 L.w_fc2, L.b_fc2 = self._T(sd[p + "mlp.c_proj.weight"].T), self._F(sd[p + "mlp.c_proj.bias"])
                 L.w_qkv_t = L.w_o_t = L.w_fc1_t = L.w_fc2_t = None
+                L.w_qkv_p = L.w_o_p = L.w_fc1_p = L.w_fc2_p = None
                 self.layers.append(L)
             self.lnf_g, self.lnf_b = self._F(sd["transformer.ln_f.weight"]), self._F(sd["transformer.ln_f.bias"])
             head = sd.get("lm_head.weight")
@@ -219,6 +224,7 @@
                 L.w_fc1, L.b_fc1 = self._T(sd[p + "fc1.weight"]), self._F(sd[p + "fc1.bias"])
                 L.w_fc2, L.b_fc2 = self._T(sd[p + "fc2.weight"]), self._F(sd[p + "fc2.bias"])
                 L.w_qkv_t = L.w_o_t = L.w_fc1_t = L.w_fc2_t = None
+                L.w_qkv_p = L.w_o_p = L.w_fc1_p = L.w_fc2_p = None
                 self.layers.append(L)
             self.lnf_g, self.lnf_b = self._F(sd[pre + "final_layer_norm.weight"]), self._F(sd[pre + "final_layer_norm.bias"])
             head = sd.get("lm_head.weight")
@@ -240,10 +246,17 @@
         q = 128 if self.weight_format == "fp8" else 64
         return (self.vocab + q - 1) // q * q
 
-    def _prepare_backward(self) -> None:
+    def _prepare_backward(self, M: int = 0, n_head_rows: int = 0) -> None:
         if self._bwd_ready:
             return
-        tr = (lambda w: w.t()) if self.weight_format == "fp8" else (lambda w: w.T.contiguous())
+        if self.weight_format == "fp8":
+            tr = lambda w: w.t()
+        else:
+            def tr(w, rows=M):
+                K, N = w.shape
+                if self.packed_weights and rows > 64 and ops.gemm_reads_packed(rows, N, K):
+                    return ops.pack_k64(w.T)
+                return w.T.contiguous()
         for L in self.layers:
             L.w_qkv_t = tr(L.w_qkv)
             L.w_o_t = tr(L.w_o)
@@ -257,7 +270,18 @@
         else:
             self.head_t = torch.zeros((E, self.vpad), device=self.device, dtype=self.dtype)
             self.head_t[:, :V] = self.head.T
+            if self.packed_weights and n_head_rows > 64 and ops.gemm_reads_packed(n_head_rows, E, self.vpad):
+                self.head_t = ops.pack_k64(self.head_t)
         self._bwd_ready = True
+
+    def _prepare_forward_packed(self) -> None:
+        if self._fwd_packed_ready:
+            return
+        for L in self.layers:
+            L.w_o_p, L.w_fc2_p = ops.pack_k64(L.w_o), ops.pack_k64(L.w_fc2)
+            if not self.fold_layernorm:
+                L.w_qkv_p, L.w_fc1_p = ops.pack_k64(L.w_qkv), ops.pack_k64(L.w_fc1)
+        self._fwd_packed_ready = True
 
     def _prepare_fold(self) -> None:
         if self._fold_ready:
@@ -267,6 +291,7 @@
                 w32 = w.float()
                 wf = (w32 * g[None, :]).to(self.dtype).contiguous()
                 setattr(L, f"w_{nm}_f", wf)
+                setattr(L, f"w_{nm}_p", ops.pack_k64(wf) if self.packed_weights else None)
                 setattr(L, f"c_{nm}", wf.float().sum(1).contiguous())
                 setattr(L, f"d_{nm}", (w32 @ be + b).contiguous())
                 del w32
@@ -293,6 +318,7 @@
             self.head = h
         self.cfg.vocab = n
         self._bwd_ready = False
+        self.head_t = None
         if self.weight_format == "fp8":
             self.head_q = Fp8Weight.quantize(self.head, self.device)
 
@@ -304,6 +330,7 @@
         if tied:
             self.head = self.wte
         self._bwd_ready = False
+        self.head_t = None
         if self.weight_format == "fp8":
             self.head_q = Fp8Weight.quantize(self.head, self.device)
 
@@ -328,6 +355,10 @@
         fold = self.fold_layernorm and M > 64
         if fold:
             self._prepare_fold()
+        packed = self.packed_weights and M > 64
+        if packed:
+            self._prepare_forward_packed()
+        lin = ops.gemm_frozen if packed else (lambda a_, w_, wp_, **kw: linear(a_, w_, **kw))
         n_slots = (E + 63) // 64
         f32 = dict(device=self.device, dtype=torch.float32)
         fuse_q = self.weight_format == "fp8" and self.fuse_quantizer
@@ -342,13 +373,13 @@
         for li, L in enumerate(self.layers):
             if st is not None:
                 mean1, rstd1 = (torch.empty(M, **f32), torch.empty(M, **f32)) if save else (None, None)
-                qkv = ops.gemm(xT, L.w_qkv_f, bias=L.d_qkv, ln_stats=st, ln_c=L.c_qkv, ln_eps=c.eps, ln_save=(mean1, rstd1) if save else None)
+                qkv = lin(xT, L.w_qkv_f, L.w_qkv_p, bias=L.d_qkv, ln_stats=st, ln_c=L.c_qkv, ln_eps=c.eps, ln_save=(mean1, rstd1) if save else None)
             else:
                 if save:
                     a, mean1, rstd1 = ln(x, L.ln1_g, L.ln1_b, True)
                 else:
                     a = ln(x, L.ln1_g, L.ln1_b, False)
-                qkv = linear(a, L.w_qkv, bias=L.b_qkv)
+                qkv = lin(a, L.w_qkv, None if fold else L.w_qkv_p, bias=L.b_qkv)
             q, k, v = qkv[:, :E], qkv[:, E:2 * E], qkv[:, 2 * E:]
             if save:
                 ctx, lse = ops.attention_fwd(q, k, v, B, H, S, S, hd, key_mask=attn_mask, causal=True, scale=scale,
@@ -358,27 +389,27 @@
             if fold:
                 x1T = torch.empty((M, E), device=self.device, dtype=T)
                 st1 = torch.empty((M, n_slots, 2), **f32)
-                x1 = ops.gemm(ctx, L.w_o, bias=L.b_o, residual=x, out_f32=True, copy_out=x1T, stats_out=st1)
+                x1 = lin(ctx, L.w_o, L.w_o_p, bias=L.b_o, residual=x, out_f32=True, copy_out=x1T, stats_out=st1)
                 mean2, rstd2 = (torch.empty(M, **f32), torch.empty(M, **f32)) if save else (None, None)
                 u = torch.empty((M, c.ffn), device=self.device, dtype=T) if save else None
-                f = ops.gemm(x1T, L.w_fc1_f, bias=L.d_fc1, act=c.act, aux_out=u, ln_stats=st1, ln_c=L.c_fc1, ln_eps=c.eps,
+                f = lin(x1T, L.w_fc1_f, L.w_fc1_p, bias=L.d_fc1, act=c.act, aux_out=u, ln_stats=st1, ln_c=L.c_fc1, ln_eps=c.eps,
                              ln_save=(mean2, rstd2) if save else None)
                 if li + 1 < len(self.layers):
                     xT = torch.empty((M, E), device=self.device, dtype=T)
                     st = torch.empty((M, n_slots, 2), **f32)
-                    x2 = ops.gemm(f, L.w_fc2, bias=L.b_fc2, residual=x1, out_f32=True, copy_out=xT, stats_out=st)
+                    x2 = lin(f, L.w_fc2, L.w_fc2_p, bias=L.b_fc2, residual=x1, out_f32=True, copy_out=xT, stats_out=st)
                 else:
-                    x2 = ops.gemm(f, L.w_fc2, bias=L.b_fc2, residual=x1, out_f32=True)
+                    x2 = lin(f, L.w_fc2, L.w_fc2_p, bias=L.b_fc2, residual=x1, out_f32=True)
             else:
-                x1 = linear(ctx, L.w_o, bias=L.b_o, residual=x, out_f32=True)
+                x1 = lin(ctx, L.w_o, L.w_o_p, bias=L.b_o, residual=x, out_f32=True)
                 if save:
                     a2, mean2, rstd2 = ln(x1, L.ln2_g, L.ln2_b, True)
                     u = torch.empty((M, c.ffn), device=self.device, dtype=T)
-                    f = linear(a2, L.w_fc1, bias=L.b_fc1, act=c.act, aux_out=u)
+                    f = lin(a2, L.w_fc1, L.w_fc1_p, bias=L.b_fc1, act=c.act, aux_out=u)
                 else:
                     a2 = ln(x1, L.ln2_g, L.ln2_b, False)
-                    f = linear(a2, L.w_fc1, bias=L.b_fc1, act=c.act)
-                x2 = linear(f, L.w_fc2, bias=L.b_fc2, residual=x1, out_f32=True)
+                    f = lin(a2, L.w_fc1, L.w_fc1_p, bias=L.b_fc1, act=c.act)
+                x2 = lin(f, L.w_fc2, L.w_fc2_p, bias=L.b_fc2, residual=x1, out_f32=True)
             if save:
                 tape.append((x, mean1, rstd1, qkv, ctx, lse, x1, mean2, rstd2, u))
             x = x2
@@ -424,7 +455,7 @@
         return lg
 
     def backward(self, tape: dict, gloss: Tensor, n_prefix_rows: int) -> Tensor:
-        self._prepare_backward()
+        self._prepare_backward(tape["M"], tape["logits"].shape[0])
         c, T = self.cfg, self.dtype
         E, H, hd = c.n_embd, c.n_head, c.head_dim
         B, S, M = tape["B"], tape["S"], tape["M"]
diff --git a/explicit-alignment-for-vqa-tasks_amd/ops.py b/explicit-alignment-for-vqa-tasks_amd/ops.py
--- a/explicit-alignment-for-vqa-tasks_amd/ops.py
+++ b/explicit-alignment-for-vqa-tasks_amd/ops.py
@@ -49,14 +49,62 @@
     return t.stride(-2) if t.dim() >= 2 else t.shape[-1]
 
 
-def gemm(a: Tensor, b: Tensor, *, a_kc: bool = True, b_kc: bool = True, bias: Optional[Tensor] = None,
+class PackedWeight:
+
+    __slots__ = ("data", "shape")
+
+    def __init__(self, data: Tensor, rows: int, cols: int):
+        self.data, self.shape = data, (int(rows), int(cols))
+
+    @property
+    def dtype(self):
+        return self.data.dtype
+
+    @property
+    def rows_padded(self) -> int:
+        return (self.shape[0] + 7) // 8 * 8
+
+
+def pack_k64(w: Tensor) -> PackedWeight:
+    _dev(w)
+    if w.dim() != 2 or w.dtype != torch.bfloat16 or w.shape[1] % 64:
+        raise _lib.EavqaError("pack_k64 takes a 2-D bfloat16 operand with K % 64 == 0")
+    R, K = w.shape
+    data = torch.empty(((R + 7) // 8 * 8) * K, device=w.device, dtype=w.dtype)
+    call("eavqa_pack_k64", BF16, R, K, _p(w), w.stride(0), w.stride(1), _p(data), _stream())
+    return PackedWeight(data, R, K)
+
+
+_reads_packed = {}
+
+
+def gemm_reads_packed(M: int, N: int, K: int) -> bool:
+    ok = _reads_packed.get((M, N, K))
+    if ok is None:
+        ok = _reads_packed[(M, N, K)] = bool(_lib.load().eavqa_gemm_reads_packed(M, N, K))
+    return ok
+
+
+def gemm_frozen(a: Tensor, w: Tensor, wp: Optional[PackedWeight], **kw) -> Tensor:
+    if wp is not None and gemm_reads_packed(a.shape[0], *wp.shape):
+        return gemm(a, wp, **kw)
+    return gemm(a, w, **kw)
+
+
+def gemm(a: Tensor, b, *, a_kc: bool = True, b_kc: bool = True, bias: Optional[Tensor] = None,
          act: str = "none", aux_in: Optional[Tensor] = None, aux_out: Optional[Tensor] = None,
          residual: Optional[Tensor] = None, out: Optional[Tensor] = None, out_f32: bool = False,
          alpha: float = 1.0, copy_out: Optional[Tensor] = None, stats_out: Optional[Tensor] = None, ln_stats: Optional[Tensor] = None,
          ln_c: Optional[Tensor] = None, ln_eps: float = 1e-5, ln_save: Optional[Tuple[Tensor, Tensor]] = None) -> Tensor:
     _dev(a)
     M, K = (a.shape if a_kc else (a.shape[1], a.shape[0]))
-    N, Kb = (b.shape if b_kc else (b.shape[1], b.shape[0]))
+    b_mode, ldb = int(b_kc), None
+    if isinstance(b, PackedWeight):
+        if not b_kc:
+            raise _lib.EavqaError("a k64-packed operand is [N, K]")
+        b_mode, ldb, (N, Kb), b = 2, b.rows_padded, b.shape, b.data
+    else:
+        N, Kb = (b.shape if b_kc else (b.shape[1], b.shape[0]))
     if K != Kb:
         raise _lib.EavqaError(f"gemm inner dims differ: {K} vs {Kb}")
     if a.dtype != b.dtype:
@@ -79,7 +127,7 @@
         if (out.dtype not in (half, torch.float32)) or (residual is not None and residual.dtype not in (half, torch.float32)):
             raise _lib.EavqaError("gemm: a float16 stream needs float16 (or float32) for both the residual and the output")
         flags |= 4
-    args = (dt, int(a_kc), int(b_kc), M, N, K, _p(a), _ld(a), _p(b), _ld(b), _p(out), _ld(out),
+    args = (dt, int(a_kc), b_mode, M, N, K, _p(a), _ld(a), _p(b), _ld(b) if ldb is None else ldb, _p(out), _ld(out),
             flags, float(alpha), _p(bias), ACT[act], _p(aux_in), _p(aux_out), _ld(aux) if aux is not None else 0,
             _p(residual), _ld(residual) if residual is not None else 0, _stream())
     if copy_out is not None or stats_out is not None or ln_stats is not None:
diff --git a/include/eavqa.h b/include/eavqa.h
--- a/include/eavqa.h
+++ b/include/eavqa.h
@@ -30,6 +30,7 @@
 const char* eavqa_strerror(int code);
 int eavqa_check_device(void);
 
+enum { EAVQA_B_K64_PACKED = 2 };
 int eavqa_gemm(int dtype, int a_kc, int b_kc, int M, int N, int K,
                const void* A, int64_t lda, const void* B, int64_t ldb,
                void* C, int64_t ldc, int out_flags, float alpha,
@@ -102,6 +103,10 @@
 int eavqa_move_rows(int dtype, int scatter, int n, int cols, const void* src, int64_t ld_src, const int32_t* idx, void* dst,
                     int64_t ld_dst, void* stream);
 int eavqa_transpose(int dtype, int rows, int cols, const void* src, int64_t ld_src, void* dst, int64_t ld_dst, void* stream);
+
+int eavqa_pack_k64(int dtype, int rows, int cols, const void* src, int64_t row_stride, int64_t col_stride, void* dst, void* stream);
+int64_t eavqa_pack_k64_offset(int rows, int cols, int row, int col);
+int eavqa_gemm_reads_packed(int M, int N, int K);
 int eavqa_colsum(int dtype, int rows, int cols, const void* x, int64_t ldx, float* out, int accumulate, void* stream);
 int eavqa_embed_assemble(int dtype, int rows, int E, const int32_t* src, const int32_t* pos,
                          const void* wte, int64_t ld_wte, const void* prefix_rows, int64_t ld_prefix,
```
